# morisUtokyo/mTR

Measured on AMD Instinct MI355X. Metric: reads/sec, 2 kb Nanopore synthetic, higher is better.
Workload: dtype int32

## Files before the change

### mtr_amd/__init__.py

```python
from __future__ import annotations

import ctypes as C
import os
from typing import List, NamedTuple, Sequence

import numpy as np

HERE = os.path.dirname(os.path.abspath(__file__))
LIB_PATH = os.environ.get("MTR_LIB", os.path.join(HERE, "libmtr_hip.so"))
MAX_PERIOD = 500
MAX_READ_LENGTH = 833333
TEXT_ASCII, TEXT_CODES = 0, 1
FASTA_TILE_BYTES = 4096
FASTA_END = {0: "eof", 1: "empty", 2: "bad", 3: "toolong"}
FASTQ_END = {**FASTA_END, 4: "format", 5: "more"}

STATUS = {0: "MTR_OK", 1: "MTR_ERR_NO_DEVICE", 2: "MTR_ERR_BAD_ARG", 3: "MTR_ERR_OOM", 4: "MTR_ERR_HIP",
          5: "MTR_ERR_OVERFLOW", 6: "MTR_ERR_DP_TOO_LARGE"}
COUNTER_NAMES = ["dp_calls", "dp_cells", "dp_rows", "revise_dp_calls", "revise_dp_cells", "kmer_tables", "kmer_lookups",
                 "ranges_candidate", "ranges_executed", "records", "di_passes", "di_positions", "traceback_steps",
                 "undefined_guards", "global_tables", "reserved",
                 "cyc_total", "cyc_dp_fwd", "cyc_dp_tb", "cyc_tab_build", "cyc_seeds", "cyc_walk", "cyc_polish", "cyc_revise_vote",
                 "cyc_slot_copy", "cyc_dp_fwd_rev", "cyc_dp_tb_rev", "cyc_k1_codes", "cyc_k1_passes", "cyc_k1_extract",
                 "cyc_k1_dedup", "cyc_k1_total",
# ... 1347 lines not shown

    def last_mode(self) -> str:
        return {0: "per-read kernel", 2: "staged chain"}.get(int(self.lib.mtr_test_last_mode(self.h)), "?")

    def fetch(self) -> List[List[Record]]:
        recs = C.POINTER(CRecord)()
        cnts = C.POINTER(C.c_int32)()
        total = C.c_int64()
        self._check(self.lib.mtr_fetch_results(self.h, C.byref(recs), C.byref(cnts), C.byref(total)), "mtr_fetch_results")
        try:
            return self._unpack(recs, cnts, self.n_reads)
        finally:
            self.lib.mtr_free_results(recs, cnts)

    def process(self, reads: Sequence[np.ndarray]) -> List[List[Record]]:
        bases, offs, lens = _flatten(reads)
        recs = C.POINTER(CRecord)()
        cnts = C.POINTER(C.c_int32)()
        total = C.c_int64()
        self.n_reads = len(reads)
        self._check(self.lib.mtr_process_batch(self.h, bases.ctypes.data, offs.ctypes.data, lens.ctypes.data, len(reads),
                                               C.byref(recs), C.byref(cnts), C.byref(total)), "mtr_process_batch")
        try:
            return self._unpack(recs, cnts, len(reads))
        finally:
            self.lib.mtr_free_results(recs, cnts)

    @staticmethod
    def _unpack(recs, cnts, n) -> List[List[Record]]:
        out, p = [], 0
        for i in range(n):
            lst = []
            for _ in range(cnts[i]):
                r = recs[p]
                p += 1
                per = r.rep_period
                lst.append(Record(r.rep_start, r.rep_end, r.repeat_len, per, r.num_freq_unit, r.num_matches, r.num_mismatches,
                                  r.num_insertions, r.num_deletions, r.kmer, r.match_gain, r.mismatch_penalty, r.indel_penalty,
                                  r.unit.decode(), tuple(r.unit_score[:max(0, min(per, MAX_PERIOD))])))
            out.append(lst)
        return out

    def upload_packed(self, reads: Sequence[np.ndarray]):
        lens = np.array([len(r) for r in reads], dtype=np.int32)
        nw = lens.astype(np.int64) // 16 + 4
        woff = np.zeros(len(reads), np.int64)
        if len(reads) > 1:
            woff[1:] = np.cumsum(nw[:-1])
        packed = np.zeros(int(nw.sum()), np.uint32)
        for i, r in enumerate(reads):
            packed[woff[i]: woff[i] + nw[i]] = pack_read(np.asarray(r, np.uint8))
        self._keep = (packed, woff, lens)
        self._check(self.lib.mtr_upload_batch_packed(self.h, packed.ctypes.data, len(packed), woff.ctypes.data, lens.ctypes.data, len(reads)),
                    "mtr_upload_batch_packed")
        self.n_reads = len(reads)

    def fetch_packed(self, limit: int = -1):
        blob, cnts = C.c_void_p(), C.c_void_p()
        nbytes, total = C.c_int64(), C.c_int64()
        self._check(self.lib.mtr_fetch_results_packed(self.h, limit, C.byref(blob), C.byref(nbytes), C.byref(cnts), C.byref(total)), "mtr_fetch_results_packed")
        n = self.n_reads if limit < 0 else min(limit, self.n_reads)
        counts = np.ctypeslib.as_array(C.cast(cnts, C.POINTER(C.c_int32)), shape=(max(n, 1),))[:n].copy() if n > 0 and cnts.value else np.zeros(0, np.int32)
        data = C.string_at(blob, nbytes.value) if nbytes.value else b""
        return data, counts

    def fetch_packed_nocopy(self):
        blob, cnts = C.c_void_p(), C.c_void_p()
        nbytes, total = C.c_int64(), C.c_int64()
        self._check(self.lib.mtr_fetch_results_packed(self.h, -1, C.byref(blob), C.byref(nbytes), C.byref(cnts), C.byref(total)), "mtr_fetch_results_packed")
        return int(nbytes.value), int(total.value)

    def fetch_via_wire(self) -> List[List[Record]]:
        data, counts = self.fetch_packed()
        total = int(counts.sum())
        recs = (CRecord * max(total, 1))()
        buf = C.create_string_buffer(data, len(data)) if data else C.create_string_buffer(1)
        st = self.lib.mtr_unpack_records(buf, len(data), total, recs)
        if st != 0:
            raise MtrError(f"mtr_unpack_records: {STATUS.get(st, st)}")
        return self._unpack(recs, counts, len(counts))

    def export_packed_device(self, device_ptr: int, capacity_bytes: int):
        counts = np.zeros(self.n_reads, np.int32)
        total, nbytes = C.c_int64(), C.c_int64()
        self._check(self.lib.mtr_export_packed_device(self.h, C.c_void_p(device_ptr), capacity_bytes, counts.ctypes.data, C.byref(total), C.byref(nbytes)),
                    "mtr_export_packed_device")
        return counts, int(total.value), int(nbytes.value)

    def first_failed_read(self) -> int:
        v = C.c_int32()
        self.lib.mtr_get_first_failed_read(self.h, C.byref(v))
        return int(v.value)

    def kernel_times_ms(self):
        kt = (CKernelTime * 10)()
        self._check(self.lib.mtr_get_kernel_times(self.h, kt, 10), "mtr_get_kernel_times")
        out = {"k1_ranges": float(kt[0].ms), "k2_units": float(kt[1].ms)}
        for i, name in enumerate(("ranges", "unit_search", "alignments", "selection", "revisions", "finish_replay")):
            if kt[2 + i].launches:
                out["chain_" + name] = float(kt[2 + i].ms)
        for i, name in enumerate(("mtr_k_revise_quads", "mtr_k_dp2_quads")):
            if kt[8 + i].launches:
                out["kernel_" + name] = float(kt[8 + i].ms)
        return out

    def counters(self):
        c = (C.c_int64 * len(COUNTER_NAMES))()
        self._check(self.lib.mtr_get_counters(self.h, c, len(COUNTER_NAMES)), "mtr_get_counters")
        return {n: int(c[i]) for i, n in enumerate(COUNTER_NAMES)}

    def test_ranges(self):
        P = C.POINTER
        pc, ps, pe, pw, pd, tot = P(C.c_int32)(), P(C.c_int32)(), P(C.c_int32)(), P(C.c_int32)(), P(C.c_uint64)(), C.c_int64()
        self._check(self.lib.mtr_test_ranges(self.h, C.byref(pc), C.byref(ps), C.byref(pe), C.byref(pw), C.byref(pd), C.byref(tot)), "mtr_test_ranges")
        out, p = [], 0
        for i in range(self.n_reads):
            out.append([(ps[p + t], pe[p + t], pw[p + t], pd[p + t]) for t in range(pc[i])])
            p += pc[i]
        for ptr in (pc, ps, pe, pw, pd):
            _libc.free(C.cast(ptr, C.c_void_p))
        return out

    def test_file_tail(self):
        P = C.POINTER
        tl, to, af = P(C.c_uint16)(), P(C.c_int64)(), P(C.c_uint8)()
        self._check(self.lib.mtr_test_file_tail(self.h, C.byref(tl), C.byref(to), C.byref(af)), "mtr_test_file_tail")
        n = self.n_reads
        try:
            tail_off = np.ctypeslib.as_array(to, shape=(n + 1,)).copy()
            m = int(tail_off[n])
            tail = np.ctypeslib.as_array(tl, shape=(m,)).copy() if m else np.zeros(0, np.uint16)
            after = np.ctypeslib.as_array(af, shape=(n, 2)).copy()
        finally:
            for a in (tl, to, af):
                _libc.free(C.cast(a, C.c_void_p))
        return tail, tail_off, after

    def test_wrap_dp(self, tasks):
        n = len(tasks)
        rd = np.array([t[0] for t in tasks], np.int32)
        qs = np.array([t[1] for t in tasks], np.int32)
        qe = np.array([t[2] for t in tasks], np.int32)
        uo = np.zeros(n + 1, np.int32)
        uo[1:] = np.cumsum([len(t[3]) for t in tasks])
        units = np.ascontiguousarray(np.concatenate([np.asarray(t[3], np.uint8) for t in tasks]))
        g = np.array([t[4] for t in tasks], np.int32)
        m = np.array([t[5] for t in tasks], np.int32)
        d = np.array([t[6] for t in tasks], np.int32)
        out = np.zeros((n, 8), np.int32)
        self._check(self.lib.mtr_test_wrap_dp(self.h, n, rd.ctypes.data, qs.ctypes.data, qe.ctypes.data, units.ctypes.data, uo.ctypes.data,
                                              g.ctypes.data, m.ctypes.data, d.ctypes.data, out.ctypes.data), "mtr_test_wrap_dp")
        return out

    DP_PASSES = {"WAVE2P": 0, "Q4": 1, "QUAD2P": 2, "FOUR1P": 3, "OCT1P": 4}

    def test_wrap_dp_pass(self, dp_pass: str, groups):
        tasks = [t for g in groups for t in g]
        n = len(tasks)
        go = np.zeros(len(groups) + 1, np.int32)
        go[1:] = np.cumsum([len(g) for g in groups])
        rd = np.array([t[0] for t in tasks], np.int32)
        qs = np.array([t[1] for t in tasks], np.int32)
        qe = np.array([t[2] for t in tasks], np.int32)
        uo = np.zeros(n + 1, np.int32)
        uo[1:] = np.cumsum([len(t[3]) for t in tasks])
        units = np.ascontiguousarray(np.concatenate([np.asarray(t[3], np.uint8) for t in tasks] + [np.zeros(1, np.uint8)]))
        g = np.array([t[4] for t in tasks], np.int32)
        m = np.array([t[5] for t in tasks], np.int32)
        d = np.array([t[6] for t in tasks], np.int32)
        out = np.zeros((max(n, 1), 2, 8), np.int32)
        self._check(self.lib.mtr_test_wrap_dp_pass(self.h, self.DP_PASSES[dp_pass], len(groups), go.ctypes.data, rd.ctypes.data, qs.ctypes.data, qe.ctypes.data,
                                                   units.ctypes.data, uo.ctypes.data, g.ctypes.data, m.ctypes.data, d.ctypes.data, out.ctypes.data),
                    "mtr_test_wrap_dp_pass")
        return out[:n]

    def set_trace(self, max_events: int):
        self._check(self.lib.mtr_set_trace(self.h, max_events), "mtr_set_trace")

    def get_trace(self) -> np.ndarray:
        ev = C.POINTER(C.c_int32)()
        n = C.c_int64()
        self._check(self.lib.mtr_get_trace(self.h, C.byref(ev), C.byref(n)), "mtr_get_trace")
        arr = np.ctypeslib.as_array(ev, shape=(max(n.value, 1), 16))[: n.value].copy()
        _libc.free(C.cast(ev, C.c_void_p))
        return arr


def _c_float_text(x) -> str:
    x = float(x)
    if x != x:
        return "-nan" if np.signbit(x) else "nan"
    if x in (float("inf"), float("-inf")):
        return "inf" if x > 0 else "-inf"
    return "%f" % x


def format_report(ids, lens, report: Report, alignments: "ReportAlignments | None" = None) -> bytes:
    def host(t):
        return t.detach().cpu().numpy() if hasattr(t, "detach") else np.asarray(t)

    read, fields, ratio = host(report.read), host(report.fields).reshape(-1, 14), host(report.ratio).astype(np.float32)
    unit_off, units = host(report.unit_off), host(report.units).tobytes()
    if alignments is not None:
        col_off, text = host(alignments.col_off), np.ascontiguousarray(host(alignments.text), np.uint8)
        text = text.reshape(3, text.size // 3)
        rows = [text[0].tobytes(), text[1].tobytes(), text[2].tobytes()]
        if len(col_off) != len(read) + 1:
            raise MtrError(f"alignments of {len(col_off) - 1} repeats for a report of {len(read)}")
    out = []
    bid = [i.encode() if isinstance(i, str) else bytes(i) for i in ids]
    for k in range(len(read)):
        r = int(read[k])
        f = [int(v) for v in fields[k]]
        cols = [str(int(lens[r])), str(f[0] + 1), str(f[1] + 1), str(f[2]), str(f[3]), str(f[4]), str(f[5]), _c_float_text(ratio[k]),
                str(f[6]), str(f[7]), str(f[8])]
        out.append(bid[r] + b"\t" + "\t".join(cols).encode() + b"\t" + units[int(unit_off[k]):int(unit_off[k + 1])] + b"\n")
        if alignments is not None:
            out.append(f"\nmatch gain = {f[10]}, mismatch penalty = {f[11]}, indel penalty = {f[12]}\n\n".encode())
            c1 = int(col_off[k + 1])
            for c in range(int(col_off[k]), c1, ALIGN_WIDTH):
                e = min(c + ALIGN_WIDTH, c1)
                out.append(rows[0][c:e] + b"\n" + rows[1][c:e] + b"\n" + rows[2][c:e] + b"\n\n")
    return b"".join(out)


_COMPLEMENT = bytes.maketrans(b"ACGT", b"TGCA")


def canonical_motif(unit):
    u = unit.encode() if isinstance(unit, str) else bytes(unit)
    p = len(u)
    if p == 0:
        return unit[:0], 0, 0
    best = None
    for strand, s in enumerate((u, u.translate(_COMPLEMENT)[::-1])):
        d = s + s
        r = min(range(p), key=lambda r: (d[r:r + p], r))
        cand = (d[r:r + p], strand, r)
        if best is None or cand[0] < best[0]:
            best = cand
    canon, strand, rotation = best
    d = next(d for d in range(1, p + 1) if p % d == 0 and canon[d:] + canon[:d] == canon)
    motif = canon[:d]
    return (motif.decode() if isinstance(unit, str) else motif), strand, rotation


def format_motif_hits(ids, lens, motifs, hits: MotifHits, min_ratio: float = 0.0, min_copies: int = 1) -> bytes:
    def host(t):
        return t.detach().cpu().numpy() if hasattr(t, "detach") else np.asarray(t)

    bmot = [v.encode() if isinstance(v, str) else bytes(v) for v in motifs]
    bid = [i.encode() if isinstance(i, str) else bytes(i) for i in ids]
    n, m = len(bid), len(bmot)
    fields, score = host(hits.fields).reshape(n, m, 8), host(hits.score).reshape(n, m)
    ratio, strand = host(hits.ratio).astype(np.float32).reshape(n, m), host(hits.strand).reshape(n, m)
    if len(lens) != n:
        raise MtrError(f"{len(lens)} lengths for {n} ids")
    shown = [(b, b.translate(_COMPLEMENT)[::-1]) for b in bmot]
    out = []
    for r, k in zip(*np.nonzero((score > 0) & (ratio >= np.float32(min_ratio)) & (fields[:, :, 3] >= min_copies))):
        f = [int(v) for v in fields[r, k]]
        cols = [str(int(lens[r])), str(f[0] + 1), str(f[1] + 1), str(f[2]), str(len(bmot[k])), str(f[3]), str(f[4]), _c_float_text(ratio[r, k]),
                str(f[5]), str(f[6]), str(f[7])]
        out.append(bid[r] + b"\t" + "\t".join(cols).encode() + b"\t" + shown[k][int(strand[r, k])] + b"\n")
    return b"".join(out)


def format_motif_loci(ids, lens, motifs, loci: MotifLoci, min_ratio: float = 0.0, min_copies: int = 1) -> bytes:
    def host(t):
        return t.detach().cpu().numpy() if hasattr(t, "detach") else np.asarray(t)

    bmot = [v.encode() if isinstance(v, str) else bytes(v) for v in motifs]
    bid = [i.encode() if isinstance(i, str) else bytes(i) for i in ids]
    n, m = len(bid), len(bmot)
    off, fields = host(loci.loci_off).reshape(-1), host(loci.fields).reshape(-1, 8)
    score, ratio, strand = host(loci.score).reshape(-1), host(loci.ratio).astype(np.float32).reshape(-1), host(loci.strand).reshape(-1)
    if len(lens) != n:
        raise MtrError(f"{len(lens)} lengths for {n} ids")
    if len(off) != n * m + 1:
        raise MtrError(f"{len(off)} offsets for {n} ids and {m} motifs: {n * m + 1} needed")
    T = int(off[-1]) if len(off) else 0
    if not (len(fields) == len(score) == len(ratio) == len(strand) == T):
        raise MtrError(f"columns of {len(fields)}, {len(score)}, {len(ratio)} and {len(strand)} rows for {T} loci")
    if int(off[0]) != 0 or (np.diff(off) < 0).any():
        raise MtrError("loci_off does not ascend from 0")
    shown = [(b, b.translate(_COMPLEMENT)[::-1]) for b in bmot]
    out = []
    for p in range(n * m):
        r, k = divmod(p, m)
        for t in range(int(off[p]), int(off[p + 1])):
            f = [int(v) for v in fields[t]]
            if not (ratio[t] >= np.float32(min_ratio) and f[3] >= min_copies):
                continue
            cols = [str(int(lens[r])), str(f[0] + 1), str(f[1] + 1), str(f[2]), str(len(bmot[k])), str(f[3]), str(f[4]), _c_float_text(ratio[t]),
                    str(f[5]), str(f[6]), str(f[7])]
            out.append(bid[r] + b"\t" + "\t".join(cols).encode() + b"\t" + shown[k][int(strand[t])] + b"\n")
    return b"".join(out)


def format_flank_hits(ids, lens, patterns, hits: FlankHits, max_dist: "int | None" = None) -> bytes:
    def host(t):
        return t.detach().cpu().numpy() if hasattr(t, "detach") else np.asarray(t)

    bpat = [v.encode() if isinstance(v, str) else bytes(v) for v in patterns]
    bid = [i.encode() if isinstance(i, str) else bytes(i) for i in ids]
    n, m = len(bid), len(bpat)
    dist, start, end, strand = (host(t).reshape(n, m) for t in hits)
# ... 300 lines not shown
```

### mtr_amd/csrc/device_util.hip.inc

```
#pragma once
#include <hip/hip_runtime.h>
#include "mtr_common.h"
#include "walk_screen.h"

#define DEVINL __device__ __forceinline__

typedef __attribute__((address_space(3))) int lds_int;
typedef __attribute__((address_space(3))) unsigned char lds_u8;

DEVINL int lane_id() { return (int)(threadIdx.x & 63u); }
__device__ long long mtr_dev_wrap_dp_size = MTRC_WRAP_DP_SIZE;
DEVINL bool dp_size_ok(int U, int rows) { return (size_t)(U + 1) * (size_t)rows + (size_t)U < (size_t)mtr_dev_wrap_dp_size; }
DEVINL int uni(int v) { return __builtin_amdgcn_readfirstlane(v); }
DEVINL long long uni64(long long v)
{
    const unsigned lo = (unsigned)__builtin_amdgcn_readfirstlane((int)(unsigned)v);
    const unsigned hi = (unsigned)__builtin_amdgcn_readfirstlane((int)(unsigned)((unsigned long long)v >> 32));
    return (long long)(((unsigned long long)hi << 32) | lo);
}
DEVINL int bcast(int v, int src) { return __shfl(v, src, 64); }
DEVINL unsigned long long lanemask_lt() { return (1ull << lane_id()) - 1ull; }
DEVINL int mbcnt(unsigned long long m)
{
    return (int)__builtin_amdgcn_mbcnt_hi((unsigned)(m >> 32), __builtin_amdgcn_mbcnt_lo((unsigned)m, 0u));
// ... 65 lines not shown
{
    return __builtin_amdgcn_update_dpp(first, v, 0x111, 0xf, 0xf, false);
}
typedef unsigned short u16x2 __attribute__((ext_vector_type(2)));
DEVINL u16x2 as_pk(unsigned v) { return __builtin_bit_cast(u16x2, v); }
DEVINL unsigned as_u32(u16x2 v) { return __builtin_bit_cast(unsigned, v); }
DEVINL unsigned pk_add(unsigned a, unsigned b) { return as_u32(as_pk(a) + as_pk(b)); }
DEVINL unsigned pk_sub(unsigned a, unsigned b) { return as_u32(as_pk(a) - as_pk(b)); }
DEVINL unsigned pk_sub_sat(unsigned a, unsigned b) { return as_u32(__builtin_elementwise_sub_sat(as_pk(a), as_pk(b))); }
DEVINL unsigned max3_u32(unsigned a, unsigned b, unsigned c) { unsigned r; asm("v_max3_u32 %0, %1, %2, %3" : "=v"(r) : "v"(a), "v"(b), "v"(c)); return r; }
DEVINL unsigned pk_max(unsigned a, unsigned b) { return as_u32(__builtin_elementwise_max(as_pk(a), as_pk(b))); }
DEVINL unsigned pk_min(unsigned a, unsigned b) { return as_u32(__builtin_elementwise_min(as_pk(a), as_pk(b))); }
template <int SH>
DEVINL unsigned lshl_or(unsigned a, unsigned b)
{
    unsigned r;
    asm("v_lshl_or_b32 %0, %1, %2, %3" : "=v"(r) : "v"(a), "n"(SH), "v"(b));
    return r;
}
DEVINL unsigned pk_nonzero(unsigned a, unsigned one_pk)
{
    unsigned r;
    asm("v_pk_min_u16 %0, %1, %2" : "=v"(r) : "v"(a), "v"(one_pk));
    return r;
}

DEVINL int shift_up1(int v, int first)
{
    return __builtin_amdgcn_update_dpp(first, v, 0x138, 0xf, 0xf, false);
}

DEVINL void scan_max_first(double &v, int &idx)
{
    int lane = lane_id();
    for (int d = 1; d < 64; d <<= 1) {
        double ov = __shfl_up(v, d, 64); int oi = __shfl_up(idx, d, 64);
        if (lane >= d && !(v > ov)) { v = ov; idx = oi; }
    }
}
DEVINL void scan_min_first(double &v, int &idx)
{
    int lane = lane_id();
    for (int d = 1; d < 64; d <<= 1) {
        double ov = __shfl_up(v, d, 64); int oi = __shfl_up(idx, d, 64);
        if (lane >= d && !(v < ov)) { v = ov; idx = oi; }
    }
}

DEVINL int next_work_item(unsigned int *counter)
{
    int t = 0;
    if (lane_id() == 0) t = (int)atomicAdd(counter, 1u);
    asm volatile("" : "+v"(t));
    return __builtin_amdgcn_readfirstlane(t);
}

#define WQ_MAX 64
#define WQ_STRIDE 64
#define WQ_WORDS (WQ_MAX * WQ_STRIDE)
struct Wq { int q, nq, tried; };
DEVINL int wq_count(unsigned n) { return n >= 131072u ? 64 : n >= 32768u ? 16 : n >= 8192u ? 4 : 1; }
DEVINL void wq_init(Wq &w, unsigned n) { w.nq = wq_count(n); w.q = (int)(blockIdx.x & (unsigned)(w.nq - 1)); w.tried = 0; }
DEVINL int wq_peek_next(unsigned int *base, unsigned n, int nq, int q, unsigned B)
{
    const int lane = lane_id();
    unsigned left = 0u;
    if (lane < nq && (unsigned)lane < n) {
        const unsigned have = (n - (unsigned)lane + (unsigned)nq - 1u) / (unsigned)nq;
        const unsigned taken = __hip_atomic_load(base + lane * WQ_STRIDE, __ATOMIC_RELAXED, __HIP_MEMORY_SCOPE_AGENT);
        left = taken < have ? have - taken : 0u;
    }
    (void)B;
    const unsigned long long m = __ballot(left != 0u);
    if (m == 0ull) return -1;
    const unsigned long long behind = q < 63 ? m & (~0ull << (q + 1)) : 0ull;
    return behind != 0ull ? __builtin_ctzll(behind) : __builtin_ctzll(m);
}
DEVINL int wq_next(unsigned int *base, unsigned n, Wq &w)
{
#ifdef MTR_WQ_PEEK
    for (;;) {
        int t = 0;
        if (lane_id() == 0) t = (int)atomicAdd(base + w.q * WQ_STRIDE, 1u);
        asm volatile("" : "+v"(t));
        const unsigned long long idx = (unsigned long long)(unsigned)__builtin_amdgcn_readfirstlane(t) * (unsigned)w.nq + (unsigned)w.q;
        if (idx < (unsigned long long)n) return (int)idx;
        if (w.nq == 1) return -1;
        const int nx = wq_peek_next(base, n, w.nq, w.q, 1u);
        if (nx < 0) return -1;
        w.q = nx;
        __builtin_amdgcn_wave_barrier();
    }
#else
    int item = -1;
    while (w.tried < w.nq) {
        int t = 0;
        if (lane_id() == 0) t = (int)atomicAdd(base + w.q * WQ_STRIDE, 1u);
        asm volatile("" : "+v"(t));
        const unsigned long long idx = (unsigned long long)(unsigned)__builtin_amdgcn_readfirstlane(t) * (unsigned)w.nq + (unsigned)w.q;
        if (idx < (unsigned long long)n) { item = (int)idx; break; }
        w.q = (w.q + 1) & (w.nq - 1); w.tried++;
        __builtin_amdgcn_wave_barrier();
    }
    return item;
#endif
}

DEVINL long long wq_next_batch(unsigned int *base, unsigned n, Wq &w, unsigned B)
{
#ifndef MTR_WQ_PEEK
    long long item = -1;
    while (w.tried < w.nq) {
        int t = 0;
        if (lane_id() == 0) t = (int)atomicAdd(base + w.q * WQ_STRIDE, B);
        asm volatile("" : "+v"(t));
        const unsigned long long idx = (unsigned long long)(unsigned)__builtin_amdgcn_readfirstlane(t) * (unsigned)w.nq + (unsigned)w.q;
        if (idx < (unsigned long long)n) { item = (long long)idx; break; }
        w.q = (w.q + 1) & (w.nq - 1); w.tried++;
        __builtin_amdgcn_wave_barrier();
    }
    return item;
#endif
    for (;;) {
        int t = 0;
        if (lane_id() == 0) t = (int)atomicAdd(base + w.q * WQ_STRIDE, B);
        asm volatile("" : "+v"(t));
        const unsigned long long idx = (unsigned long long)(unsigned)__builtin_amdgcn_readfirstlane(t) * (unsigned)w.nq + (unsigned)w.q;
        if (idx < (unsigned long long)n) return (long long)idx;
        if (w.nq == 1) return -1;
        const int nx = wq_peek_next(base, n, w.nq, w.q, B);
        if (nx < 0) return -1;
        w.q = nx;
        __builtin_amdgcn_wave_barrier();
    }
}

DEVINL void loop_join() { __builtin_amdgcn_wave_barrier(); }

DEVINL void count_add(unsigned long long *counters, int which, long long v)
{
    if (lane_id() == 0) atomicAdd(&counters[which], (unsigned long long)v);
}
DEVINL void wc_add(unsigned long long *wc, int which, long long v)
{
    if (lane_id() == 0) wc[which] += (unsigned long long)v;
}
#ifdef MTR_PROFILE
DEVINL unsigned long long clk() { return __builtin_amdgcn_s_memtime(); }
DEVINL void wc_time(unsigned long long *wc, int which, unsigned long long t0) { wc_add(wc, which, (long long)(clk() - t0)); }
#else
DEVINL unsigned long long clk() { return 0ull; }
DEVINL void wc_time(unsigned long long *, int, unsigned long long) {}
#endif
#ifdef MTR_PROFILE_WALK_FMT
#define wc_time_aux(wc, which, t0) do { } while (0)
#else
#define wc_time_aux(wc, which, t0) wc_time(wc, which, t0)
#endif
DEVINL void wc_flush(unsigned long long *wc, unsigned long long *global)
{
    const int lane = lane_id();
    __builtin_amdgcn_wave_barrier();
    if (lane < CNT_N) { unsigned long long v = wc[lane]; if (v) atomicAdd(&global[lane], v); wc[lane] = 0ull; }
    __builtin_amdgcn_wave_barrier();
}
DEVINL void set_status(int32_t *status, int code)
{
    if (lane_id() == 0) atomicCAS(status, 0, code);
}
DEVINL void wave_sync_mem()
{
    __builtin_amdgcn_fence(__ATOMIC_RELEASE, "workgroup");
    __builtin_amdgcn_wave_barrier();
    __builtin_amdgcn_fence(__ATOMIC_ACQUIRE, "workgroup");
}
```

### mtr_amd/csrc/dp_quad.hip.inc

```
#pragma once
#include "device_util.hip.inc"

struct DpQuad {
    const uint32_t *pk[4];
    long long wlim[4];
    int base[4], rows[4], U[4];
    const uint8_t *unit[4];
    int n;
    int G[4], MM[4], D[4];
};
#define DPQ_SCALE 4
#define DPQ_FITS_SC(SC, rows, U, G, D) ((long)(SC) * ((long)(rows) * (long)(G) + (long)(D) * ((long)(U) + 2)) < 65000L)
#define DPQ_FITS(rows, U, G, D) DPQ_FITS_SC(DPQ_SCALE, rows, U, G, D)
#define DPQ_COLS(U) (((U) + 15) >> 4)
#define DPQ_COLS64(U) (((U) + 63) >> 6)
#define DPQ_ROW_BYTES_G(GL, C) ((GL) * (C))
#define DPQ_DP_BYTES_G(GL, C, maxrows) ((size_t)(maxrows) * DPQ_ROW_BYTES_G(GL, C) + 16)
#define DPQ_ROW_BYTES(C) DPQ_ROW_BYTES_G(16, C)
#define DPQ_DP_BYTES(C, maxrows) DPQ_DP_BYTES_G(16, C, maxrows)
#define DPQ_BLOCK_BYTES(C, maxrows) (4 * DPQ_DP_BYTES(C, maxrows))
#define DPQP_DP_BYTES_G(GL, C, maxrows) ((size_t)(((maxrows) + 1) >> 1) * DPQ_ROW_BYTES_G(GL, C) + 16)
#define DPQP_DP_BYTES(C, maxrows) DPQP_DP_BYTES_G(16, C, maxrows)
#define DPQP_BLOCK_BYTES(C, maxrows) (4 * DPQP_DP_BYTES(C, maxrows))

template <int C, int GL = 16, int SC = DPQ_SCALE>
DEVINL void dp_forward2p_g16(const DpQuad &q, int G0, int MM0, int D0, int G1, int MM1, int D1, uint8_t *cells, int maxrows, int (&best)[4][2][3])
{
    static_assert(C >= 1 && C <= 8 && (GL == 16 || GL == 64) && (SC == 1 || SC == 4), "columns per lane, lanes per DP, score scale");
    constexpr int NG = 64 / GL;
    const int lane = lane_id();
    const int g = lane / GL, l = lane % GL;
    unsigned Gpk = SC * ((unsigned)G0 | ((unsigned)G1 << 16)), MMpk = SC * ((unsigned)MM0 | ((unsigned)MM1 << 16)), Dpk = SC * ((unsigned)D0 | ((unsigned)D1 << 16));
    unsigned ONE = 0x00010001u, TWO = 0x00020002u, FOUR = 0x00040004u, SEL_HI = 0x07060100u, C8 = 0x00080008u;
    asm volatile("" : "+v"(ONE), "+v"(TWO), "+v"(FOUR), "+v"(SEL_HI), "+v"(C8));
    unsigned SEL_K0 = 0x0c040100u, SEL_K1 = 0x0c040302u, SEL_S = 0x05040100u, SEL_LO = 0x05040100u, SEL_P1 = 0x07060302u, K4N = ~0x00040004u;
    asm volatile("" : "+s"(MMpk), "+s"(Dpk), "+s"(SEL_K0), "+s"(SEL_K1), "+s"(SEL_S), "+s"(SEL_LO), "+s"(SEL_P1), "+s"(K4N));
    int Ul = q.U[0], basel = q.base[0], rowsl = q.rows[0]; const uint8_t *up_ = q.unit[0]; const uint32_t *pkl = q.pk[0]; long long wl = q.wlim[0];
    if (g == 1) { Ul = q.U[1]; basel = q.base[1]; rowsl = q.rows[1]; up_ = q.unit[1]; pkl = q.pk[1]; wl = q.wlim[1]; }
    if (g == 2) { Ul = q.U[2]; basel = q.base[2]; rowsl = q.rows[2]; up_ = q.unit[2]; pkl = q.pk[2]; wl = q.wlim[2]; }
    if (g == 3) { Ul = q.U[3]; basel = q.base[3]; rowsl = q.rows[3]; up_ = q.unit[3]; pkl = q.pk[3]; wl = q.wlim[3]; }
    if (g >= q.n) { Ul = 0; rowsl = 0; }
    unsigned ubw[2] = { 0x04040404u, 0x04040404u };
    unsigned Kc[C], KGc[C];
#pragma unroll
    for (int c = 0; c < C; c++) {
        const int j = l * C + c + 1;
        if (j <= Ul) ubw[c >> 2] = (ubw[c >> 2] & ~(0xffu << (8 * (c & 3)))) | ((unsigned)(up_[j - 1] & 3) << (8 * (c & 3)));
        Kc[c] = SC * ((unsigned)(D0 * (c + 1)) | ((unsigned)(D1 * (c + 1)) << 16));
        KGc[c] = Kc[c] + Gpk;
    }
    const unsigned Dlane = SC * ((unsigned)(D0 * l * C) | ((unsigned)(D1 * l * C) << 16));
    {
        int landed = lane_val((int)(ubw[0] ^ ubw[1]), 0);
        asm volatile("" :: "s"(landed));
    }
    const int lU = Ul > 0 ? (Ul - 1) / C : 0, rU = Ul > 0 ? (Ul - 1) % C : 0;
    const int hu_addr = (g * GL + lU) << 2;
    const int lUs = GL == 64 ? uni(lU) : 0;
    bool is_r[C];
#pragma unroll
    for (int c = 0; c < C; c++) is_r[c] = rU == c;
    const bool lane0 = l == 0;
    const int grp_addr = (g * GL) << 2;
    constexpr bool BKP = SC == 4;
    static_assert(65000 / DPQ_SCALE <= 0x7FFF, "DPQ_FITS must keep the rows of an SC = 4 pass within the 15 bits of the pair keys");
    constexpr int NBK = BKP ? (C + 1) / 2 : C;
    unsigned P[C], bk0[NBK], bk1[NBK];
#pragma unroll
    for (int c = 0; c < C; c++) P[c] = 0u;
#pragma unroll
    for (int c = 0; c < NBK; c++) { bk0[c] = 0u; bk1[c] = 0u; }
    unsigned wrapv = 0u;
    int next_done = maxrows + 1;
#pragma unroll
    for (int h = 0; h < NG; h++) { const int r = h < q.n ? q.rows[h] : 0; if (r < next_done) next_done = r; }
    if (rowsl <= 0) { ubw[0] = 0x04040404u; ubw[1] = 0x04040404u; }
    uint8_t *crow = cells + (size_t)g * DPQ_DP_BYTES_G(GL, C, maxrows) + (size_t)l * C;
    int i = 1;
    constexpr int CHUNK = 16 * GL - 16;
    for (int t0 = 0; t0 < maxrows; t0 += CHUNK) {
        const int pos0 = basel + 1 + t0;
        long long w0 = (long long)(pos0 >> 4) + l;
        long long w1 = w0 + 1;
        if (w0 > wl - 1) w0 = wl - 1;
        if (w1 > wl - 1) w1 = wl - 1;
        if (w0 < 0) w0 = 0;
        if (w1 < 0) w1 = 0;
        const uint32_t wa = pkl[w0], wb = pkl[w1];
        const unsigned sh = 2u * (unsigned)(pos0 & 15);
        const uint32_t A = (uint32_t)(((((unsigned long long)wa) << 32) | (unsigned long long)wb) >> (32u - sh));
        {
            int landed = lane_val((int)A, 0);
            asm volatile("" :: "s"(landed));
        }
        const int i_chunk_end = t0 + CHUNK < maxrows ? t0 + CHUNK : maxrows;
        for (int wd = 0; i <= i_chunk_end; wd++) {
            const uint32_t wcur = (uint32_t)__builtin_amdgcn_ds_bpermute(grp_addr + (wd << 2), (int)A);
            const int i_w_end = i + 15 < i_chunk_end ? i + 15 : i_chunk_end;
            int bsh = 30;
#pragma unroll 1
            for (; i <= i_w_end; i++, bsh -= 2) {
                if (i > next_done) {
                    if (i > rowsl) { ubw[0] = 0x04040404u; ubw[1] = 0x04040404u; }
                    next_done = maxrows + 1;
#pragma unroll
                    for (int h = 0; h < NG; h++) { const int r = h < q.n ? q.rows[h] : 0; if (r >= i && r < next_done) next_done = r; }
                }
                const unsigned xi = __builtin_amdgcn_ubfe(wcur, (unsigned)bsh, 2u);
                const unsigned inv_i = 0xFFFFu - (unsigned)i;
                unsigned s[C], t1s[C];
                bool mt[C], nh[C];
                unsigned sprev = 0u;
                bool nhp = true;
                const unsigned diag0 = GL == 16 ? (unsigned)row_shift_up1((int)P[C - 1], (int)wrapv) : (unsigned)shift_up1((int)P[C - 1], (int)wrapv);
#pragma unroll
                for (int c = 0; c < C; c++) {
                    const unsigned diag = c == 0 ? diag0 : P[c - 1];
                    const unsigned upv = P[c];
                    const bool m = ((ubw[c >> 2] >> (8 * (c & 3))) & 0xffu) == xi;
                    const unsigned t1 = pk_sub_sat(diag, MMpk), t2 = pk_sub_sat(upv, Dpk);
                    const unsigned gnm = pk_max(t1, t2) + Kc[c];
                    const unsigned gm = diag + KGc[c];
                    const unsigned ch = pk_max(gnm, sprev);
                    const unsigned sc = m ? gm : ch;
                    s[c] = sc; t1s[c] = t1; mt[c] = m;
                    nhp = nhp && !m; nh[c] = nhp;
                    sprev = sc;
                }
                const unsigned long long hm = __ballot(!nhp);
                const unsigned seg = (unsigned)mbcnt(hm >> 1);
                const unsigned sout = sprev + Dlane;
                unsigned k0 = __builtin_amdgcn_perm(seg, sout, SEL_K0);
                unsigned k1 = __builtin_amdgcn_perm(seg, sout, SEL_K1);
                if (GL == 16) scan_max_u32_x2_row16(k0, k1); else scan_max_u32_x2(k0, k1);
                const unsigned S = __builtin_amdgcn_perm(k1, k0, SEL_S);
                const unsigned e = (GL == 16 ? (unsigned)row_shift_up1((int)S, 0) : (unsigned)shift_up1((int)S, 0)) - Dlane;
                unsigned f[8];
#pragma unroll
                for (int c = C; c < 8; c++) f[c] = 0u;
                unsigned hgp = e;
#pragma unroll
                for (int c = 0; c < C; c++) {
                    const unsigned mx = pk_max(s[c], e);
                    const unsigned hg = nh[c] ? mx : s[c];
                    const unsigned H = hg - Kc[c];
                    const unsigned nz = pk_nonzero(H, ONE);
                    const unsigned nx = pk_nonzero(H - t1s[c], SC == 4 ? TWO : ONE);
                    const unsigned nd = pk_nonzero(hg - hgp, SC == 4 ? FOUR : ONE);
                    unsigned fl;
                    if (SC == 4) asm("v_or3_b32 %0, %1, %2, %3" : "=v"(fl) : "v"(nz), "v"(nx), "v"(nd));
                    else fl = lshl_or<1>(nx, lshl_or<2>(nd, nz));
                    fl = mt[c] ? C8 : fl;
                    f[c] = fl;
                    if (!BKP) {
                        const unsigned q0 = (H << 16) | inv_i, q1 = __builtin_amdgcn_perm(H, inv_i, SEL_HI);
                        bk0[c] = q0 > bk0[c] ? q0 : bk0[c];
                        bk1[c] = q1 > bk1[c] ? q1 : bk1[c];
                    }
                    P[c] = H;
                    hgp = hg;
                }
                if (BKP) {
                    const unsigned r0 = (0x7FFFu - (unsigned)i) << 1, r1 = r0 | 1u;
#pragma unroll
                    for (int c = 0; c + 1 < C; c += 2) {
                        const unsigned a0 = (P[c] << 16) | r1, b0 = (P[c + 1] << 16) | r0;
                        const unsigned a1 = __builtin_amdgcn_perm(P[c], r1, SEL_HI), b1 = __builtin_amdgcn_perm(P[c + 1], r0, SEL_HI);
                        bk0[c >> 1] = max3_u32(bk0[c >> 1], a0, b0);
                        bk1[c >> 1] = max3_u32(bk1[c >> 1], a1, b1);
                    }
                    if (C & 1) {
                        const unsigned a0 = (P[C - 1] << 16) | r1, a1 = __builtin_amdgcn_perm(P[C - 1], r1, SEL_HI);
                        bk0[C >> 1] = a0 > bk0[C >> 1] ? a0 : bk0[C >> 1];
                        bk1[C >> 1] = a1 > bk1[C >> 1] ? a1 : bk1[C >> 1];
                    }
                }
                unsigned hsel = P[0];
#pragma unroll
                for (int c = 1; c < C; c++) hsel = is_r[c] ? P[c] : hsel;
                wrapv = GL == 64 ? (unsigned)__builtin_amdgcn_readlane((int)hsel, lUs) : (unsigned)__builtin_amdgcn_ds_bpermute(hu_addr, (int)hsel);
                {
                    unsigned nd0 = pk_nonzero(pk_sub(pk_add(P[0], Dpk), wrapv), SC == 4 ? FOUR : ONE);
                    if (SC != 4) nd0 <<= 2;
                    unsigned f0;
                    asm("v_and_or_b32 %0, %1, %2, %3" : "=v"(f0) : "v"(f[0]), "s"(K4N), "v"(nd0));
                    f[0] = (lane0 && !mt[0]) ? f0 : f[0];
                }
                const unsigned F01 = lshl_or<8>(f[1], f[0]), F23 = lshl_or<8>(f[3], f[2]);
                unsigned lo = lshl_or<4>(__builtin_amdgcn_perm(F23, F01, SEL_P1), __builtin_amdgcn_perm(F23, F01, SEL_LO));
                if (C > 4) {
                    const unsigned F45 = C > 5 ? lshl_or<8>(f[5], f[4]) : f[4], F67 = C > 7 ? lshl_or<8>(f[7], f[6]) : f[6];
                    unsigned hi = lshl_or<4>(__builtin_amdgcn_perm(F67, F45, SEL_P1), __builtin_amdgcn_perm(F67, F45, SEL_LO));
                    if (C < 8) {
                        const unsigned nlo = (unsigned)__builtin_amdgcn_update_dpp(0, (int)lo, 0x130, 0xf, 0xf, false);
                        hi = lshl_or<8 * (C > 4 && C < 8 ? C - 4 : 0)>(nlo, hi);
                    }
                    *(uint2 *)crow = make_uint2(lo, hi);
                } else if (C == 1) {
                    *crow = (uint8_t)lo;
                } else {
                    if (C < 4) {
                        const unsigned nlo = (unsigned)__builtin_amdgcn_update_dpp(0, (int)lo, 0x130, 0xf, 0xf, false);
                        lo = lshl_or<8 * (C < 4 ? C : 0)>(nlo, lo);
                    }
                    *(uint32_t *)crow = lo;
                }
                crow += DPQ_ROW_BYTES_G(GL, C);
                loop_join();
            }
            loop_join();
        }
        loop_join();
    }
#pragma unroll
    for (int d = 0; d < 2; d++) {
        int v = 0, vi = 0, vj = 0;
#pragma unroll
        for (int t = 0; t < NBK; t++) {
            const unsigned bk = d == 0 ? bk0[t] : bk1[t];
            const int c = BKP ? 2 * t + 1 - (int)(bk & 1u) : t;
            const int j = l * C + c + 1;
            const int bvc = (int)(bk >> 16), bic = BKP ? (int)(0x7FFFu - ((bk & 0xFFFFu) >> 1)) : (int)(0xFFFFu - (bk & 0xFFFFu));
            if (j <= Ul && (bvc > v || (bvc == v && bvc > 0 && bic < vi))) { v = bvc; vi = bic; vj = j; }
        }
        for (int dd = GL / 2; dd > 0; dd >>= 1) {
            const int ov = __shfl_xor(v, dd, 64), oi = __shfl_xor(vi, dd, 64), oj = __shfl_xor(vj, dd, 64);
            const bool take = (ov > v) || (ov == v && ov > 0 && (oi < vi || (oi == vi && oj < vj)));
            if (take) { v = ov; vi = oi; vj = oj; }
        }
#pragma unroll
        for (int h = 0; h < NG; h++) { best[h][d][0] = lane_val(v, GL * h) / SC; best[h][d][1] = lane_val(vi, GL * h); best[h][d][2] = lane_val(vj, GL * h); }
    }
}


DEVINL unsigned u16_max(unsigned a, unsigned b) { unsigned r; asm("v_max_u16_e32 %0, %1, %2" : "=v"(r) : "v"(a), "v"(b)); return r; }
DEVINL unsigned u16_min(unsigned a, unsigned b) { unsigned r; asm("v_min_u16_e32 %0, %1, %2" : "=v"(r) : "v"(a), "v"(b)); return r; }
DEVINL unsigned u16_sub_sat(unsigned a, unsigned b) { unsigned r; asm("v_sub_u16_e64 %0, %1, %2 clamp" : "=v"(r) : "v"(a), "v"(b)); return r; }
DEVINL unsigned u16_sub(unsigned a, unsigned b) { unsigned r; asm("v_sub_u16_e32 %0, %1, %2" : "=v"(r) : "v"(a), "v"(b)); return r; }
DEVINL unsigned scan_max_u32_row16(unsigned a)
{
    unsigned s;
#define MTR_SCAN_STEP(ctrl) s = (unsigned)__builtin_amdgcn_update_dpp(0, (int)a, ctrl, 0xf, 0xf, false); a = s > a ? s : a;
    MTR_SCAN_STEP(0x111) MTR_SCAN_STEP(0x112) MTR_SCAN_STEP(0x114) MTR_SCAN_STEP(0x118)
#undef MTR_SCAN_STEP
    return a;
}
template <int C, int GL = 16, int SC = DPQ_SCALE, bool PAIR = false>
DEVINL void dp_forward1p_g16(const DpQuad &q, uint8_t *cells, int maxrows, int (&best)[4][3])
{
    static_assert(C >= 1 && C <= 8 && (GL == 16 || GL == 64) && (SC == 1 || SC == 4), "columns per lane, lanes per DP, score scale");
    constexpr int NG = 64 / GL;
    const int lane = lane_id();
    const int g = lane / GL, l = lane % GL;
    unsigned ONE = 1u, TWO = 2u, FOUR = 4u, EIGHT = 8u;
    asm volatile("" : "+v"(ONE), "+v"(TWO), "+v"(FOUR), "+v"(EIGHT));
    int Ul = q.U[0], basel = q.base[0], rowsl = q.rows[0]; const uint8_t *up_ = q.unit[0]; const uint32_t *pkl = q.pk[0]; long long wl = q.wlim[0];
    int Gl = q.G[0], MMl = q.MM[0], Dl = q.D[0];
    if (g == 1) { Ul = q.U[1]; basel = q.base[1]; rowsl = q.rows[1]; up_ = q.unit[1]; pkl = q.pk[1]; wl = q.wlim[1]; Gl = q.G[1]; MMl = q.MM[1]; Dl = q.D[1]; }
    if (g == 2) { Ul = q.U[2]; basel = q.base[2]; rowsl = q.rows[2]; up_ = q.unit[2]; pkl = q.pk[2]; wl = q.wlim[2]; Gl = q.G[2]; MMl = q.MM[2]; Dl = q.D[2]; }
    if (g == 3) { Ul = q.U[3]; basel = q.base[3]; rowsl = q.rows[3]; up_ = q.unit[3]; pkl = q.pk[3]; wl = q.wlim[3]; Gl = q.G[3]; MMl = q.MM[3]; Dl = q.D[3]; }
    if (g >= q.n) { Ul = 0; rowsl = 0; }
    const unsigned Gs = SC * (unsigned)Gl, MMs = SC * (unsigned)MMl, Ds = SC * (unsigned)Dl;
    unsigned ubw[2] = { 0x04040404u, 0x04040404u };
    unsigned Dj[C], GDj[C];
#pragma unroll
    for (int c = 0; c < C; c++) {
        const int j = l * C + c + 1;
        if (j <= Ul) ubw[c >> 2] = (ubw[c >> 2] & ~(0xffu << (8 * (c & 3)))) | ((unsigned)(up_[j - 1] & 3) << (8 * (c & 3)));
        Dj[c] = Ds * (unsigned)j;
        GDj[c] = Dj[c] + Gs;
    }
    {
        int landed = lane_val((int)(ubw[0] ^ ubw[1]), 0);
        asm volatile("" :: "s"(landed));
    }
    const int lU = Ul > 0 ? (Ul - 1) / C : 0, rU = Ul > 0 ? (Ul - 1) % C : 0;
    const int hu_addr = (g * GL + lU) << 2;
    const int lUs = GL == 64 ? uni(lU) : 0;
    bool is_r[C];
#pragma unroll
    for (int c = 0; c < C; c++) is_r[c] = rU == c;
    const bool lane0 = l == 0;
    const int grp_addr = (g * GL) << 2;
    constexpr bool BKP = SC == 4;
    constexpr int NBK = BKP ? (C + 1) / 2 : C;
    unsigned P[C], bk[NBK];
#pragma unroll
    for (int c = 0; c < C; c++) P[c] = 0u;
#pragma unroll
    for (int c = 0; c < NBK; c++) bk[c] = 0u;
    unsigned wrapv = 0u;
    int next_done = maxrows + 1;
#pragma unroll
    for (int h = 0; h < NG; h++) { const int r = h < q.n ? q.rows[h] : 0; if (r < next_done) next_done = r; }
    if (rowsl <= 0) { ubw[0] = 0x04040404u; ubw[1] = 0x04040404u; }
    uint8_t *crow = cells + (size_t)g * (PAIR ? DPQP_DP_BYTES_G(GL, C, maxrows) : DPQ_DP_BYTES_G(GL, C, maxrows)) + (size_t)l * C;
    unsigned loP = 0u, hiP = 0u;
    auto store_cells = [&](unsigned lo, unsigned hi) {
        if (C > 4) {
            if (C < 8) {
                const unsigned nlo = (unsigned)__builtin_amdgcn_update_dpp(0, (int)lo, 0x130, 0xf, 0xf, false);
                hi |= nlo << (8 * (C > 4 && C < 8 ? C - 4 : 0));
            }
            *(uint2 *)crow = make_uint2(lo, hi);
        } else if (C == 1) {
            *crow = (uint8_t)lo;
        } else {
            if (C < 4) {
                const unsigned nlo = (unsigned)__builtin_amdgcn_update_dpp(0, (int)lo, 0x130, 0xf, 0xf, false);
                lo |= nlo << (8 * (C < 4 ? C : 0));
            }
            *(uint32_t *)crow = lo;
        }
        crow += DPQ_ROW_BYTES_G(GL, C);
    };
    int i = 1;
    constexpr int CHUNK = 16 * GL - 16;
    for (int t0 = 0; t0 < maxrows; t0 += CHUNK) {
        const int pos0 = basel + 1 + t0;
        long long w0 = (long long)(pos0 >> 4) + l;
        long long w1 = w0 + 1;
        if (w0 > wl - 1) w0 = wl - 1;
        if (w1 > wl - 1) w1 = wl - 1;
        if (w0 < 0) w0 = 0;
        if (w1 < 0) w1 = 0;
        const uint32_t wa = pkl[w0], wb = pkl[w1];
        const unsigned sh = 2u * (unsigned)(pos0 & 15);
        const uint32_t A = (uint32_t)(((((unsigned long long)wa) << 32) | (unsigned long long)wb) >> (32u - sh));
        {
            int landed = lane_val((int)A, 0);
            asm volatile("" :: "s"(landed));
        }
        const int i_chunk_end = t0 + CHUNK < maxrows ? t0 + CHUNK : maxrows;
        for (int wd = 0; i <= i_chunk_end; wd++) {
            const uint32_t wcur = (uint32_t)__builtin_amdgcn_ds_bpermute(grp_addr + (wd << 2), (int)A);
            const int i_w_end = i + 15 < i_chunk_end ? i + 15 : i_chunk_end;
            int bsh = 30;
#pragma unroll 1
            for (; i <= i_w_end; i++, bsh -= 2) {
                if (i > next_done) {
                    if (i > rowsl) { ubw[0] = 0x04040404u; ubw[1] = 0x04040404u; }
                    next_done = maxrows + 1;
#pragma unroll
                    for (int h = 0; h < NG; h++) { const int r = h < q.n ? q.rows[h] : 0; if (r >= i && r < next_done) next_done = r; }
                }
                const unsigned xi = __builtin_amdgcn_ubfe(wcur, (unsigned)bsh, 2u);
                const unsigned inv_i = 0xFFFFu - (unsigned)i;
                unsigned s[C], t1s[C];
                bool mt[C], nh[C];
                unsigned sprev = 0u;
                bool nhp = true;
                const unsigned diag0 = GL == 16 ? (unsigned)row_shift_up1((int)P[C - 1], (int)wrapv) : (unsigned)shift_up1((int)P[C - 1], (int)wrapv);
#pragma unroll
                for (int c = 0; c < C; c++) {
                    const unsigned diag = c == 0 ? diag0 : P[c - 1];
                    const unsigned upv = P[c];
                    const bool m = ((ubw[c >> 2] >> (8 * (c & 3))) & 0xffu) == xi;
                    const unsigned t1 = u16_sub_sat(diag, MMs), t2 = u16_sub_sat(upv, Ds);
                    const unsigned gnm = u16_max(t1, t2) + Dj[c];
                    const unsigned gm = diag + GDj[c];
                    const unsigned ch = u16_max(gnm, sprev);
                    const unsigned sc = m ? gm : ch;
                    s[c] = sc; t1s[c] = t1; mt[c] = m;
                    nhp = nhp && !m; nh[c] = nhp;
                    sprev = sc;
                }
                const unsigned long long hm = __ballot(!nhp);
                const unsigned seg = (unsigned)mbcnt(hm >> 1);
                const unsigned S = (GL == 16 ? scan_max_u32_row16((seg << 16) | sprev) : scan_max_u32((seg << 16) | sprev)) & 0xFFFFu;
                const unsigned e = GL == 16 ? (unsigned)row_shift_up1((int)S, 0) : (unsigned)shift_up1((int)S, 0);
                unsigned f[8];
#pragma unroll
                for (int c = C; c < 8; c++) f[c] = 0u;
                unsigned hgp = e;
#pragma unroll
                for (int c = 0; c < C; c++) {
                    const unsigned mx = u16_max(s[c], e);
                    const unsigned hg = nh[c] ? mx : s[c];
                    const unsigned H = hg - Dj[c];
                    const unsigned nz = u16_min(H, ONE);
                    const unsigned nx = u16_min(H - t1s[c], SC == 4 ? TWO : ONE);
                    const unsigned nd = u16_min(hg - hgp, SC == 4 ? FOUR : ONE);
                    unsigned fl = SC == 4 ? (nz | nx | nd) : (nz | (nx << 1) | (nd << 2));
// ... 295 lines not shown
```

### mtr_amd/csrc/dp_test.hip.inc

```
#pragma once
#include "dp_wrap.hip.inc"

struct DpPassArgs {
    DpTestArgs t;
    int32_t pass, n_groups;
    const int32_t *group_off;
    long long packed_words;
};

DEVINL void dpt_clear(DpRes &o) { o.stop_i = 0; o.end_i = 0; o.mat = o.mis = o.ins = o.del = o.scanned = 0; o.end_j = 0; }
DEVINL void dpt_store(const DpPassArgs &a, int task, int p, int qs, int U, const DpRes &o)
{
    if (lane_id() == 0) {
        int32_t *r = a.t.out8 + ((size_t)task * 2 + (size_t)p) * 8;
        r[0] = qs + o.stop_i + 1; r[1] = qs + o.end_i; r[2] = o.end_i - o.stop_i; r[3] = U > 0 ? o.scanned / U : 0;
        r[4] = o.mat; r[5] = o.mis; r[6] = o.ins; r[7] = o.del;
    }
}
template <int FMT>
DEVINL void dpt_traceback(const DpPassArgs &a, const uint32_t *pk, int qs, int U, const uint8_t *cells, int psel, int rstride, const int (&best)[3],
                          DpRes &o, unsigned long long *wc)
{
    dpt_clear(o);
    const int bv = uni(best[0]), bi = uni(best[1]), bj = uni(best[2]);
    if (bv > 0) {
        dp_traceback<0, FMT>(pk, qs, U, cells, psel, rstride, bi, bj, nullptr, nullptr, nullptr, o, wc);
        if (o.stop_i < 0) { dpt_clear(o); set_status(a.t.status, DEV_ERR_DP_TOO_LARGE); }
    }
}

__global__ __launch_bounds__(64, MTR_DP2_WAVES_PER_SIMD) void mtr_k_dp_test_waves(DpPassArgs a)
{
    __shared__ unsigned long long s_cnt[CNT_N];
    if (lane_id() < CNT_N) s_cnt[lane_id()] = 0ull;
    uint8_t *sc = a.t.scratch + (size_t)blockIdx.x * a.t.scratch_per_wave;
    for (;;) {
        const int grp = next_work_item(a.t.work_counter);
        if (grp >= a.n_groups) break;
        const int t0 = uni(a.group_off[grp]), n = uni(a.group_off[grp + 1]) - t0;
        const int rd = uni(a.t.read_idx[t0]);
        const uint32_t *pk = a.t.b.packed + uni64(a.t.b.woff[rd]);
        const int qs = uni(a.t.qs[t0]), rows = uni(a.t.qe[t0]) - qs + 1;
        if (a.pass == MTR_TEST_PASS_WAVE2P) {
            const int uo = uni(a.t.unit_off[t0]), U = uni(a.t.unit_off[t0 + 1]) - uo;
            const uint8_t *unit = a.t.units + uo;
            DpRes o[2];
            bool ok;
            if (dp_wrap2_fits(rows, U, a.t.dp16_max_rows)) ok = dp_wrap2(pk, qs, rows, unit, U, 1, 1, 3, 1, 3, 1, sc, a.t.cells_cap, o, s_cnt, a.t.dp16_max_rows);
            else {
                ok = dp_wrap(pk, qs, rows, unit, U, 1, 1, 3, sc, a.t.cells_cap, 0, nullptr, nullptr, nullptr, o[0], s_cnt, a.t.dp16_max_rows);
                ok = dp_wrap(pk, qs, rows, unit, U, 1, 3, 1, sc, a.t.cells_cap, 0, nullptr, nullptr, nullptr, o[1], s_cnt, a.t.dp16_max_rows) && ok;
            }
            if (!ok) set_status(a.t.status, DEV_ERR_DP_TOO_LARGE);
            dpt_store(a, t0, 0, qs, U, o[0]); dpt_store(a, t0, 1, qs, U, o[1]);
        } else {
            Dp4 q; q.n = n;
            size_t off = 0;
#pragma unroll
            for (int g = 0; g < 4; g++) {
                const bool on = g < n;
                const int tg = t0 + (on ? g : 0);
                const int uo = uni(a.t.unit_off[tg]);
                q.U[g] = on ? uni(a.t.unit_off[tg + 1]) - uo : 1; q.unit[g] = a.t.units + uo;
                q.off[g] = on ? off : 0;
                if (on) off += (size_t)rows * (size_t)q.U[g];
            }
            int best[4][2][3];
            dp_forward2p_q4(pk, qs, rows, q, 1, 1, 3, 1, 3, 1, sc, best);
            wave_sync_mem();
#pragma unroll
            for (int g = 0; g < 4; g++) {
                if (g < n) {
                    for (int p = 0; p < 2; p++) {
                        DpRes o;
                        dpt_traceback<1>(a, pk, qs, q.U[g], sc + q.off[g], p, q.U[g], best[g][p], o, s_cnt);
                        dpt_store(a, t0 + g, p, qs, q.U[g], o);
                        loop_join();
                    }
                }
            }
        }
        wave_sync_mem();
        loop_join();
    }
    wc_flush(s_cnt, a.t.counters);
}

template <int C>
__global__ __launch_bounds__(64, 4) void mtr_k_dp_test_quads(DpPassArgs a)
{
    __shared__ unsigned long long s_cnt[CNT_N];
    if (lane_id() < CNT_N) s_cnt[lane_id()] = 0ull;
    uint8_t *cells = a.t.scratch + (size_t)blockIdx.x * a.t.scratch_per_wave;
    for (;;) {
        const int grp = next_work_item(a.t.work_counter);
        if (grp >= a.n_groups) break;
        const int t0 = uni(a.group_off[grp]), n = uni(a.group_off[grp + 1]) - t0;
        DpQuad q; q.n = n;
        int maxrows = 0;
#pragma unroll
        for (int g = 0; g < 4; g++) {
            const int tg = t0 + (g < n ? g : 0);
            const int rd = uni(a.t.read_idx[tg]), uo = uni(a.t.unit_off[tg]);
            q.pk[g] = a.t.b.packed + uni64(a.t.b.woff[rd]);
            q.wlim[g] = a.packed_words - uni64(a.t.b.woff[rd]);
            q.base[g] = uni(a.t.qs[tg]); q.rows[g] = g < n ? uni(a.t.qe[tg]) - q.base[g] + 1 : 0;
            q.U[g] = uni(a.t.unit_off[tg + 1]) - uo; q.unit[g] = a.t.units + uo;
            q.G[g] = 1; q.MM[g] = 1; q.D[g] = 1;
            maxrows = q.rows[g] > maxrows ? q.rows[g] : maxrows;
        }
        int best[4][2][3];
        dp_forward2p_g16<C>(q, 1, 1, 3, 1, 3, 1, cells, maxrows, best);
        wave_sync_mem();
#pragma unroll
        for (int g = 0; g < 4; g++) {
            if (g < n) {
                for (int p = 0; p < 2; p++) {
                    DpRes o;
                    dpt_traceback<1>(a, q.pk[g], q.base[g], q.U[g], cells + g * DPQ_DP_BYTES(C, maxrows), p, DPQ_ROW_BYTES(C), best[g][p], o, s_cnt);
                    dpt_store(a, t0 + g, p, q.base[g], q.U[g], o);
                    loop_join();
                }
            }
        }
        wave_sync_mem();
        loop_join();
    }
    wc_flush(s_cnt, a.t.counters);
}

__global__ __launch_bounds__(64, MTR_WAVES_PER_SIMD) void mtr_k_dp_test_rev(DpPassArgs a)
{
    __shared__ unsigned long long s_cnt[CNT_N];
    if (lane_id() < CNT_N) s_cnt[lane_id()] = 0ull;
    uint8_t *cells = a.t.scratch + (size_t)blockIdx.x * a.t.scratch_per_wave;
    for (;;) {
        const int grp = next_work_item(a.t.work_counter);
        if (grp >= a.n_groups) break;
        const int t0 = uni(a.group_off[grp]), n = uni(a.group_off[grp + 1]) - t0;
        DpOct q; q.n = n;
        int maxrows = 0, maxU = 0;
#pragma unroll 1
        for (int g = 0; g < RQ_SLOTS; g++) { q.pk[g] = a.t.b.packed; q.wlim[g] = 1; q.base[g] = 0; q.rows[g] = 0; q.U[g] = 0; q.unit[g] = cells; q.G[g] = 1; q.MM[g] = 1; q.D[g] = 1; }
#pragma unroll 1
        for (int k = 0; k < n; k++) {
            const int tg = t0 + k;
            const int rd = uni(a.t.read_idx[tg]), uo = uni(a.t.unit_off[tg]);
            q.pk[k] = a.t.b.packed + uni64(a.t.b.woff[rd]); q.wlim[k] = a.packed_words - uni64(a.t.b.woff[rd]);
            q.base[k] = uni(a.t.qs[tg]); q.rows[k] = uni(a.t.qe[tg]) - q.base[k] + 1;
            q.U[k] = uni(a.t.unit_off[tg + 1]) - uo; q.unit[k] = a.t.units + uo;
            q.G[k] = uni(a.t.gain[tg]); q.MM[k] = uni(a.t.mism[tg]); q.D[k] = uni(a.t.indel[tg]);
            maxrows = q.rows[k] > maxrows ? q.rows[k] : maxrows; maxU = q.U[k] > maxU ? q.U[k] : maxU;
        }
        const int Cq = DPQ_COLS(maxU);
        int best[RQ_SLOTS][3];
        for (int g = 0; g < RQ_SLOTS; g++) { best[g][0] = 0; best[g][1] = 0; best[g][2] = 0; }
        if (a.pass == MTR_TEST_PASS_FOUR1P) st_fwd1p_four(Cq, q, cells, maxrows, best); else st_fwd1p_any(Cq, q, cells, maxrows, best);
        wave_sync_mem();
#pragma unroll 1
        for (int k = 0; k < n; k++) {
            int bk[3] = { best[0][0], best[0][1], best[0][2] };
#pragma unroll
            for (int h = 1; h < RQ_SLOTS; h++) if (k == h) { bk[0] = best[h][0]; bk[1] = best[h][1]; bk[2] = best[h][2]; }
            const int tg = t0 + k;
            const int rd = uni(a.t.read_idx[tg]), qs = uni(a.t.qs[tg]), U = uni(a.t.unit_off[tg + 1]) - uni(a.t.unit_off[tg]);
            DpRes o;
            dpt_traceback<3>(a, a.t.b.packed + uni64(a.t.b.woff[rd]), qs, U, cells + (size_t)k * DPQP_DP_BYTES(Cq, maxrows), 0, DPQ_ROW_BYTES(Cq), bk, o, s_cnt);
            dpt_store(a, tg, 0, qs, U, o);
            loop_join();
        }
        wave_sync_mem();
        loop_join();
    }
    wc_flush(s_cnt, a.t.counters);
}
```

### mtr_amd/csrc/k3_staged.hip.inc

```
#pragma once
#include "k2_units.hip.inc"
#include "dp_quad.hip.inc"

#define ST_QCLASSES 8
#define ST_QROWBINS 2048
#define ST_QSUB 8
#define ST_NBINS (ST_QCLASSES * ST_QROWBINS * ST_QSUB)
#define ST_QUMAX 128

struct StItemHdr {
    int32_t n_slots; uint32_t run_mask, found_mask; int32_t min_k, max_k;
    int32_t rd, t, qs, qe, w, item, stride;
    long long pad0, pad1;
};
struct StEnt { int32_t period, k, dir, dpi; };
struct StK { int32_t state, slot; int32_t rr[14]; long long rev_off; };
struct StRev { long long block; int32_t k, slot; int32_t rr[14]; long long leader; int32_t ri, pad[3]; };
#define ST_REV_BYTES ((long long)sizeof(StRev) + K2_SLOT_UNIT + 4ll * K2_SLOT_SCORE)
struct StDpItem { int32_t rd, qs, rows, U; long long unit_off, codes_off; int32_t best[6]; int32_t pad[2]; };
static_assert(sizeof(StItemHdr) == 64 && sizeof(StEnt) == 16 && sizeof(StDpItem) == 64 && sizeof(StK) == 72 && sizeof(StRev) == 96, "staged layouts");

struct StagedArgs {
    int32_t n_reads;
    int64_t *item_off; int32_t *n_items;
    int4 *item_tab; int32_t item_cap;
    uint8_t *arena; long long arena_cap;
    long long *kc_items; int32_t kc_cap;
    long long *rb_items;
    StDpItem *dp; int32_t dp_cap;
    unsigned *bin_count; int32_t *dp_bin, *dp_rank;
    int32_t *bin_start; int32_t *sorted; int32_t sorted_cap; int32_t *quad_cls;
    int32_t quad_min;
    DevRecord *cand; int32_t cand_cap; unsigned *n_cand; int32_t *cand_flag;
    unsigned *work;
    int4 *cont; int32_t cont_cap;
    int32_t k_first;
    long long *rev_items; int32_t rev_cap; unsigned *n_rev;
    int32_t *wv_items; int32_t *dp_res;
    int32_t nsub;
    int32_t two_pass, pass, defer_w;
    int32_t pass_shuffle;
    int32_t test_flags;
    int8_t *item_pass; int32_t *pass_list[2]; unsigned *n_pass[2];
    int32_t *re2;
    int32_t walk_screen; int32_t *walk_list; int32_t walk_cap; unsigned *n_walk;
};

#define ST_NCLS 8
#define ST_CLS_STRIDE 64
DEVINL int st_cost_class(int rows)
{
    if (rows < 128) return 0;
    const int c = (31 - __builtin_clz((unsigned)rows)) - 6;
    return c > ST_NCLS - 1 ? ST_NCLS - 1 : c;
}
#define ST_Q_DP 16
#define ST_Q_WK 24
#define ST_Q_REV 32
#define ST_Q_QUAD 40
#define ST_Q_POLISH 56
#define ST_N_QUEUES 64
#define ST_WQ(s, j) ((s).work + (size_t)(j) * WQ_WORDS)
DEVINL bool st_staged_overflowed(const K2Args &a) { return uni(*(volatile int32_t *)a.status) == DEV_ERR_STAGED_OVERFLOW; }

#define ST_SL_DP 1
#define ST_SL_ARENA 2
#define ST_SL_KC 3
#define ST_SL_REV 4
#define ST_SL_RB 58
#define ST_DPI_DUP 0x40000000
DEVINL int st_sl_cont(int cls) { return cls < 2 ? 6 + cls : cls == 2 ? 9 : 11 + (cls - 3); }
#define ST_SL_WV 48
DEVINL unsigned *st_sub(const StagedArgs &s, int slot, int q) { return ST_WQ(s, slot) + (size_t)q * WQ_STRIDE; }
DEVINL int st_my_sub(const StagedArgs &s) { return (int)(blockIdx.x & (unsigned)(s.nsub - 1)); }
DEVINL long long st_reserve(const StagedArgs &s, int slot, long long cap, unsigned n)
{
    const int q = st_my_sub(s);
    const long long per = cap / s.nsub;
    unsigned got = 0;
    if (lane_id() == 0) got = atomicAdd(st_sub(s, slot, q), n);
    got = (unsigned)uni((int)got);
    if ((long long)got + (long long)n > per) return -1;
    return (long long)q * per + (long long)got;
}
DEVINL long long st_reserve_bytes(const StagedArgs &s, long long bytes)
{
    const int q = st_my_sub(s);
    const long long per = (s.arena_cap / s.nsub) & ~15ll;
    unsigned long long got = 0;
    if (lane_id() == 0) got = atomicAdd((unsigned long long *)st_sub(s, ST_SL_ARENA, q), (unsigned long long)bytes);
    got = (unsigned long long)uni64((long long)got);
    if ((long long)got + bytes > per) return -1;
    return (long long)q * per + (long long)got;
}
struct WqS { int q, tried, cnt; };
DEVINL long long wqs_init(WqS &w, const StagedArgs &s, int cslot, long long cap)
{
    const int lane = lane_id();
    const long long per = cap / s.nsub;
    unsigned c = lane < s.nsub ? *st_sub(s, cslot, lane) : 0u;
    if ((long long)c > per) c = (unsigned)per;
    w.cnt = (int)c; w.q = st_my_sub(s); w.tried = 0;
    return wave_sum_i64((long long)c);
}
DEVINL long long wqs_next(const StagedArgs &s, int qslot, long long cap, WqS &w)
{
    const long long per = cap / s.nsub;
#ifndef MTR_WQ_PEEK
    while (w.tried < s.nsub) {
        const int n_q = lane_val(w.cnt, w.q);
        if (n_q > 0) {
            int t = 0;
            if (lane_id() == 0) t = (int)atomicAdd(ST_WQ(s, qslot) + (size_t)w.q * WQ_STRIDE, 1u);
            asm volatile("" : "+v"(t));
            t = __builtin_amdgcn_readfirstlane(t);
            if (t < n_q) return (long long)w.q * per + (long long)t;
        }
        w.q = (w.q + 1) & (s.nsub - 1); w.tried++;
        __builtin_amdgcn_wave_barrier();
    }
    return -1;
#endif
    for (;;) {
        const int n_q = lane_val(w.cnt, w.q);
        if (n_q > 0) {
            int t = 0;
            if (lane_id() == 0) t = (int)atomicAdd(ST_WQ(s, qslot) + (size_t)w.q * WQ_STRIDE, 1u);
            asm volatile("" : "+v"(t));
            t = __builtin_amdgcn_readfirstlane(t);
            if (t < n_q) return (long long)w.q * per + (long long)t;
        }
        if (s.nsub == 1) return -1;
        unsigned left = 0u;
        if (lane_id() < s.nsub) {
            const unsigned taken = __hip_atomic_load(ST_WQ(s, qslot) + (size_t)lane_id() * WQ_STRIDE, __ATOMIC_RELAXED, __HIP_MEMORY_SCOPE_AGENT);
            left = taken < (unsigned)w.cnt ? (unsigned)w.cnt - taken : 0u;
        }
        const unsigned long long m = __ballot(left != 0u);
        if (m == 0ull) return -1;
        const unsigned long long behind = w.q < 63 ? m & (~0ull << (w.q + 1)) : 0ull;
        w.q = behind != 0ull ? __builtin_ctzll(behind) : __builtin_ctzll(m);
        __builtin_amdgcn_wave_barrier();
    }
}
DEVINL long long st_pad16(long long x) { return (x + 15) & ~15ll; }

__global__ __launch_bounds__(1024) void mtr_k_items(const int32_t *r_count, StagedArgs s)
{
    __shared__ long long part[1024];
    const int tid = (int)threadIdx.x, n = s.n_reads;
    const int per = (n + 1023) / 1024;
    const int lo = tid * per, hi = lo + per < n ? lo + per : n;
    long long sum = 0;
    for (int i = lo; i < hi; i++) sum += r_count[i];
    part[tid] = sum;
    __syncthreads();
    for (int d = 1; d < 1024; d <<= 1) {
        const long long v = tid >= d ? part[tid - d] : 0;
        __syncthreads();
        part[tid] += v;
        __syncthreads();
// ... 272 lines not shown
                    for (int k = k_last + 1; k <= max_k; k++)
                        if ((alive >> (k - min_k)) & 1u) s.cont[q++] = make_int4((int)(unsigned)(base & 0xffffffffll), (int)(base >> 32), k, bound);
                }
                wave_sync_mem();
                st_park_entries(c, s, base, st, min_k, stride, n_slots, maxU);
            }
        }
        loop_join();
        }
        loop_join();
    }
    wc_flush(s_cnt, a.counters);
}

__global__ __launch_bounds__(64, MTR_WAVES_PER_SIMD) void mtr_k_walks_k(K2Args a, StagedArgs s)
{
    __shared__ __attribute__((aligned(16))) int s_arena[MTR_ARENA_INTS];
    __shared__ unsigned long long s_cnt[CNT_N];
    int *s_keys = s_arena, *s_seeds = s_arena + K2_TAB_CAP, *s_stage = s_seeds + MTRC_MAX_SEEDS + 4;
    const int lane = lane_id();
    if (lane < CNT_N) s_cnt[lane] = 0ull;
    if (st_staged_overflowed(a)) return;
    K2Ctx c;
    c.a = &a; c.wc = s_cnt; c.staged_walks = true;
#ifdef MTR_PROFILE_WALK_FMT
    c.prof_kernel = 1;
#endif
    c.sc = a.scratch + (size_t)blockIdx.x * a.scratch_per_wave;
    c.y = k2_layout(a.Lmax, a.cells_cap);
    c.lds_keys = (lds_int *)s_keys; c.seeds = (lds_int *)s_seeds; c.stage = (lds_int *)s_stage;
    c.ties = (int *)(c.sc + c.y.ties); c.fresh = c.ties + MTRC_MAX_TIEBREAKS;
    for (int cls = ST_NCLS - 1; cls >= 0; cls--) {
    WqS wq;
    if (wqs_init(wq, s, st_sl_cont(cls), s.cont_cap) == 0) continue;
    for (;;) {
        const long long wi = wqs_next(s, ST_Q_WK + cls, s.cont_cap, wq);
        if (wi < 0) break;
        int4 rec = make_int4(0, 0, 0, 0);
        if (lane == 0) rec = s.cont[(size_t)cls * (size_t)s.cont_cap + wi];
        const long long base = (long long)(((unsigned long long)(unsigned)uni(rec.y) << 32) | (unsigned)uni(rec.x));
        const int k = uni(rec.z), bound = uni(rec.w);
        StItemHdr *h = (StItemHdr *)(s.arena + base);
        c.rd = uni(h->rd);
        const int qs = uni(h->qs), qe = uni(h->qe), w = uni(h->w), min_k = uni(h->min_k), n_slots = uni(h->n_slots), stride = uni(h->stride);
        c.L = uni(a.b.lens[c.rd]);
        c.pk = a.b.packed + uni64(a.b.woff[c.rd]);
        c.memo_n = 0; c.memo_qs = c.memo_qe = -1; c.memo_U = 0;
        RangeP1 st;
#ifdef MTR_PROFILE_WALK_WIDTH
        const unsigned long long t_w = clk();
#endif
        k2_range_walks(c, qs, qe, w, st, k, k, bound);
#ifdef MTR_PROFILE_WALK_WIDTH
        { const int wd_ = qe - qs + 1; wc_time(c.wc, wd_ < 32 ? CNT_SPARE43 : wd_ < 64 ? CNT_SPARE44 : wd_ < 128 ? CNT_SPARE45 : wd_ < 256 ? CNT_SPARE46 : CNT_SPARE55, t_w); }
#endif
        if (lane == 0) { if (st.run_mask) atomicOr(&h->run_mask, st.run_mask); if (st.found_mask) atomicOr(&h->found_mask, st.found_mask); }
        if (st.n_ent > 0) st_park_entries(c, s, base, st, min_k, stride, n_slots, st_max_unit(qs, qe));
        loop_join();
    }
    loop_join();
    }
    wc_flush(s_cnt, a.counters);
}

DEVINL unsigned st_rotl(unsigned x, int r) { return (x << r) | (x >> (32 - r)); }
__global__ __launch_bounds__(64) void mtr_k_gather(K2Args a, StagedArgs s)
{
    const int lane = lane_id();
    if (st_staged_overflowed(a)) return;
    WqS wq; (void)wqs_init(wq, s, ST_SL_KC, s.kc_cap);
    for (;;) {
        const long long wi = wqs_next(s, 8, s.kc_cap, wq);
        if (wi < 0) break;
        const long long base = uni64(s.kc_items[wi]);
        StItemHdr *h = (StItemHdr *)(s.arena + base);
        StEnt *en = (StEnt *)(h + 1);
        int hv = 0;
        if (lane < 12) hv = ((const int32_t *)h)[lane];
        const int n_slots = lane_val(hv, 0), min_k = lane_val(hv, 3), rd = lane_val(hv, 5), qs = lane_val(hv, 7), qe = lane_val(hv, 8), stride = lane_val(hv, 11);
        const unsigned found_mask = (unsigned)lane_val(hv, 2);
        const int rows = qe - qs + 1;
        const int ns = n_slots < 32 ? n_slots : 32;
        int Ue = 0, ke = min_k;
        if (lane < ns) { Ue = en[lane].period; ke = en[lane].k; }
        uint8_t *slot0 = s.arena + base + (long long)sizeof(StItemHdr) + (long long)sizeof(StEnt) * n_slots;
        const bool cand_l = lane < ns && Ue >= MTRC_MIN_PERIOD && ((found_mask >> (ke - min_k)) & 1u);
        const unsigned candm = (unsigned)__ballot(cand_l);
        if (candm == 0u) { loop_join(); continue; }
        unsigned h1 = 0u, h2 = 0u;
        if (cand_l) {
            const uint32_t *uw = (const uint32_t *)(slot0 + (long long)lane * stride);
            const int nw = (Ue + 3) >> 2;
            const uint32_t last_mask = (Ue & 3) ? ((1u << (8 * (Ue & 3))) - 1u) : 0xffffffffu;
            int q = 0;
            for (; q + 4 <= nw; q += 4) {
                uint32_t w0 = uw[q], w1 = uw[q + 1], w2 = uw[q + 2], w3 = uw[q + 3];
                if (q + 4 == nw) w3 &= last_mask;
                h1 = st_rotl((h1 ^ w0) * 0x9E3779B1u, 13); h2 = (h2 + w0) * 0x85EBCA77u; h2 ^= h2 >> 15;
                h1 = st_rotl((h1 ^ w1) * 0x9E3779B1u, 13); h2 = (h2 + w1) * 0x85EBCA77u; h2 ^= h2 >> 15;
                h1 = st_rotl((h1 ^ w2) * 0x9E3779B1u, 13); h2 = (h2 + w2) * 0x85EBCA77u; h2 ^= h2 >> 15;
                h1 = st_rotl((h1 ^ w3) * 0x9E3779B1u, 13); h2 = (h2 + w3) * 0x85EBCA77u; h2 ^= h2 >> 15;
            }
            for (; q < nw; q++) {
                uint32_t w0 = uw[q];
                if (q + 1 == nw) w0 &= last_mask;
                h1 = st_rotl((h1 ^ w0) * 0x9E3779B1u, 13); h2 = (h2 + w0) * 0x85EBCA77u; h2 ^= h2 >> 15;
            }
        }
        unsigned want = 0u;
        int dupof_l = -1;
        for (unsigned cm = candm; cm != 0u; cm &= cm - 1u) {
            const int e = __builtin_ctz(cm);
            const int U = lane_val(Ue, e);
            const unsigned e1 = (unsigned)lane_val((int)h1, e), e2 = (unsigned)lane_val((int)h2, e);
            const uint8_t *ub = slot0 + (long long)e * stride;
            bool dup = false;
            for (unsigned sm = (unsigned)__ballot(lane < ns && Ue == U && h1 == e1 && h2 == e2) & want; sm != 0u && !dup; sm &= sm - 1u) {
                const int j = __builtin_ctz(sm);
                const uint8_t *u2 = slot0 + (long long)j * stride;
                bool diff = false;
                for (int q = lane; q < U; q += 64) diff = diff || (u2[q] != ub[q]);
                dup = __ballot(diff) == 0ull;
                if (dup && lane == e) dupof_l = j;
                loop_join();
            }
            if (!dup) want |= 1u << e;
            loop_join();
        }
        const int n_want = __builtin_popcount(want);
        const bool fits16 = rows <= DP2P_MAX_ROWS && rows <= a.dp16_max_rows;
        const bool grouping = fits16 && s.dp_cap < (1 << 28);
        const bool isq = s.quad_min > 0 && fits16 && Ue <= ST_QUMAX && DPQ_FITS(rows, Ue, 1, 3) && dp_size_ok(Ue, rows);
        const unsigned quadm = (unsigned)__ballot(isq) & want, smallm = (unsigned)__ballot(!isq && grouping && Ue <= 16) & want;
        const unsigned restm = want & ~smallm & ~quadm;
        const int n_small = __builtin_popcount(smallm), n_quad = __builtin_popcount(quadm), n_entries = (n_small + 3) / 4 + (n_want - n_small - n_quad);
        const int cls = st_cost_class(rows);
        const long long dres = st_reserve(s, ST_SL_DP, s.dp_cap, (unsigned)n_want);
        const long long wres = n_entries > 0 ? st_reserve(s, ST_SL_WV + cls, s.dp_cap, (unsigned)n_entries) : 0;
        if (dres < 0 || wres < 0) { set_status(a.status, DEV_ERR_STAGED_OVERFLOW); loop_join(); continue; }
        const unsigned di0 = (unsigned)dres, wv0 = (unsigned)wres;
        int dpi_l = -1;
        if (lane < 32 && ((want >> lane) & 1u)) {
            const unsigned below = (1u << lane) - 1u;
            const bool is_small = (smallm >> lane) & 1u, is_quad = (quadm >> lane) & 1u;
            const int nth = is_small ? __builtin_popcount(smallm & below) : is_quad ? n_small + __builtin_popcount(quadm & below) : n_small + n_quad + __builtin_popcount(restm & below);
            const unsigned di = di0 + (unsigned)nth;
            dpi_l = (int)di;
            StDpItem *d = s.dp + di;
            d->rd = rd; d->qs = qs; d->rows = rows; d->U = Ue; d->unit_off = (long long)(slot0 + (long long)lane * stride - s.arena); d->codes_off = -1;
            for (int q = 0; q < 6; q++) d->best[q] = 0;
            d->pad[0] = ke; d->pad[1] = cls;
            if (is_quad) {
                int rb = ST_QROWBINS - 1 - (rows >> 3); if (rb < 0) rb = 0;
                const int bin = ((8 - DPQ_COLS(Ue)) * ST_QROWBINS + rb) * ST_QSUB + (int)(blockIdx.x & (ST_QSUB - 1));
                s.dp_bin[di] = bin; s.dp_rank[di] = (int32_t)atomicAdd(s.bin_count + bin, 1u);
            } else {
                s.dp_bin[di] = -1;
                if (is_small) {
                    if ((nth & 3) == 0) {
                        const int members = n_small - nth < 4 ? n_small - nth : 4;
                        s.wv_items[(size_t)cls * (size_t)s.dp_cap + wv0 + (unsigned)(nth >> 2)] = (int32_t)(di | ((unsigned)(members - 1) << 28));
                    }
                } else s.wv_items[(size_t)cls * (size_t)s.dp_cap + wv0 + (unsigned)((n_small + 3) / 4 + (nth - n_small - n_quad))] = (int32_t)di;
            }
            en[lane].dpi = (int32_t)di;
        }
        {
            const int od = __shfl(dpi_l, dupof_l >= 0 ? dupof_l : 0, 64);
            if (dupof_l >= 0 && od >= 0 && s.dp_cap < ST_DPI_DUP) en[lane].dpi = (int32_t)(od | ST_DPI_DUP);
        }
        wave_sync_mem();
        loop_join();
    }
}

__global__ __launch_bounds__(1024) void mtr_k_qbins(StagedArgs s, int force)
{
    __shared__ int tot[1024];
    __shared__ int cls_start[ST_QCLASSES + 1], cls_n[ST_QCLASSES];
    const int t = (int)threadIdx.x;
    constexpr int PER = ST_NBINS / 1024, TPC = ST_QROWBINS * ST_QSUB / PER;
    static_assert(PER % 4 == 0, "a thread's bins are read four at a time");
    int sum = 0;
    for (int r = 0; r < PER; r += 4) { const uint4 v = *(const uint4 *)(s.bin_count + t * PER + r); sum += (int)(v.x + v.y + v.z + v.w); }
    tot[t] = sum;
    __syncthreads();
    for (int d = 1; d < 1024; d <<= 1) {
        const int v = t >= d ? tot[t - d] : 0;
        __syncthreads();
        tot[t] += v;
        __syncthreads();
    }
    if (t == 0) {
        int off = 0;
        for (int c = 0; c < ST_QCLASSES; c++) {
            const int n = tot[(c + 1) * TPC - 1] - (c > 0 ? tot[c * TPC - 1] : 0);
            cls_start[c] = off; cls_n[c] = n;
            off += (n + 3) & ~3;
        }
        cls_start[ST_QCLASSES] = off;
        const bool use = s.quad_min > 0 && (force || tot[1023] >= s.quad_min) && off <= s.sorted_cap;
        for (int c = 0; c <= ST_QCLASSES; c++) s.quad_cls[c] = use ? cls_start[c] : 0;
        s.quad_cls[ST_QCLASSES + 1] = use ? 1 : 0;
        if (use) for (int c = 0; c < ST_QCLASSES; c++) for (int q = cls_start[c] + cls_n[c]; q < cls_start[c + 1]; q++) s.sorted[q] = -1;
    }
    __syncthreads();
    const int c = t / TPC;
    int off = cls_start[c] + (tot[t] - sum) - (c > 0 ? tot[c * TPC - 1] : 0);
    for (int r = 0; r < PER; r += 4) {
        const uint4 v = *(const uint4 *)(s.bin_count + t * PER + r);
        int4 o; o.x = off; o.y = off + (int)v.x; o.z = o.y + (int)v.y; o.w = o.z + (int)v.z;
        *(int4 *)(s.bin_start + t * PER + r) = o;
        off = o.w + (int)v.w;
        *(uint4 *)(s.bin_count + t * PER + r) = make_uint4(0u, 0u, 0u, 0u);
    }
}
__global__ void mtr_k_qscatter(StagedArgs s, int32_t *status)
{
    if (*(volatile int32_t *)status == DEV_ERR_STAGED_OVERFLOW) return;
    const unsigned per = (unsigned)(s.dp_cap / s.nsub);
    const bool use = s.quad_cls[ST_QCLASSES + 1] != 0;
    for (unsigned i = blockIdx.x * blockDim.x + threadIdx.x; i < per * (unsigned)s.nsub; i += gridDim.x * blockDim.x) {
        if (i % per >= *st_sub(s, ST_SL_DP, (int)(i / per))) continue;
        if (s.dp_bin[i] < 0) continue;
        if (use) {
            const int slot = s.bin_start[s.dp_bin[i]] + s.dp_rank[i];
            if (slot >= 0 && slot < s.sorted_cap) s.sorted[slot] = (int32_t)i;
        } else {
            const int cls = s.dp[i].pad[1];
            const unsigned wper = (unsigned)(s.dp_cap / s.nsub), wq_ = blockIdx.x & (unsigned)(s.nsub - 1);
            const unsigned w = atomicAdd(st_sub(s, ST_SL_WV + cls, (int)wq_), 1u);
            if (w < wper) s.wv_items[(size_t)cls * (size_t)s.dp_cap + (size_t)wq_ * wper + w] = (int32_t)i;
            else atomicCAS(status, 0, DEV_ERR_STAGED_OVERFLOW);
        }
    }
}

__global__ void mtr_k_rscatter(StagedArgs s, int32_t *status)
{
    if (*(volatile int32_t *)status == DEV_ERR_STAGED_OVERFLOW) return;
    const unsigned per = (unsigned)(s.rev_cap / s.nsub);
    for (unsigned i = blockIdx.x * blockDim.x + threadIdx.x; i < per * (unsigned)s.nsub; i += gridDim.x * blockDim.x) {
        if (i % per >= *st_sub(s, ST_SL_REV, (int)(i / per))) continue;
        if (s.dp_bin[i] < 0) continue;
        const int slot = s.bin_start[s.dp_bin[i]] + s.dp_rank[i];
        if (slot >= 0 && slot < s.sorted_cap) s.sorted[slot] = (int32_t)i;
    }
}

DEVINL void st_dp2_waves_body(K2Ctx &c, const K2Args &a, const StagedArgs &s)
{
    const int lane = lane_id();
    for (int cls = ST_NCLS - 1; cls >= 0; cls--) {
    WqS wq;
    if (wqs_init(wq, s, ST_SL_WV + cls, s.dp_cap) == 0) continue;
    for (;;) {
        const long long wi = wqs_next(s, ST_Q_DP + cls, s.dp_cap, wq);
        if (wi < 0) break;
        const unsigned ent = (unsigned)uni(s.wv_items[(size_t)cls * (size_t)s.dp_cap + wi]);
        const int di0 = (int)(ent & 0x0FFFFFFFu), members = (int)(ent >> 28) + 1;
        const StDpItem *d0 = s.dp + di0;
        c.rd = uni(d0->rd);
        c.L = uni(a.b.lens[c.rd]);
        c.pk = a.b.packed + uni64(a.b.woff[c.rd]);
        const int qs = uni(d0->qs), rows = uni(d0->rows);
        if (members > 1 && dp_batch_fits(c, rows)) {
            Dp4 q; q.n = members;
            int kk[4];
#pragma unroll
            for (int g = 0; g < 4; g++) {
                const StDpItem *dg = s.dp + di0 + (g < members ? g : 0);
                q.U[g] = uni(dg->U); kk[g] = uni(dg->pad[0]); q.unit[g] = s.arena + uni64(dg->unit_off); q.off[g] = 0;
            }
            dp_two_params_q4(c, qs, qs + rows - 1, q, kk, [&](int g, const RR &r, bool) {
                int *o = s.dp_res + (size_t)(di0 + g) * 16;
                if (lane == 0) {
                    o[0] = r.rep_start; o[1] = r.rep_end; o[2] = r.repeat_len; o[3] = r.period; o[4] = r.copies; o[5] = r.mat; o[6] = r.mis;
                    o[7] = r.ins; o[8] = r.del; o[9] = r.kmer; o[10] = r.G; o[11] = r.MM; o[12] = r.D;
                }
            });
        } else {
        for (int g = 0; g < members; g++) {
        const int di = di0 + g;
        const StDpItem *d = s.dp + di;
        const int U = uni(d->U);
        RR r; rr_clear(r); r.period = U; r.kmer = uni(d->pad[0]);
        dp_two_params_unit(c, qs, qs + rows - 1, r, s.arena + uni64(d->unit_off));
        int *o = s.dp_res + (size_t)di * 16;
        if (lane == 0) {
            o[0] = r.rep_start; o[1] = r.rep_end; o[2] = r.repeat_len; o[3] = r.period; o[4] = r.copies; o[5] = r.mat; o[6] = r.mis;
            o[7] = r.ins; o[8] = r.del; o[9] = r.kmer; o[10] = r.G; o[11] = r.MM; o[12] = r.D;
        }
        loop_join();
        }
        }
        loop_join();
    }
    loop_join();
    }
}
#ifndef MTR_DP2_WAVES_PER_SIMD
#define MTR_DP2_WAVES_PER_SIMD 8
#endif
__global__ __launch_bounds__(64, MTR_DP2_WAVES_PER_SIMD) void mtr_k_dp2_waves(K2Args a, StagedArgs s)
{
    __shared__ unsigned long long s_cnt[CNT_N];
    const int lane = lane_id();
    if (lane < CNT_N) s_cnt[lane] = 0ull;
    if (st_staged_overflowed(a)) return;
    K2Ctx c;
    c.a = &a; c.wc = s_cnt;
    c.sc = a.scratch + (size_t)blockIdx.x * a.scratch_per_wave;
    c.y = k2_layout(a.Lmax, a.cells_cap);
    c.lds_keys = nullptr; c.seeds = nullptr; c.stage = nullptr; c.ties = nullptr; c.fresh = nullptr;
    st_dp2_waves_body(c, a, s);
    wc_flush(s_cnt, a.counters);
}

template <int C>
DEVINL void st_quad_run(K2Ctx &c, const K2Args &a, const StagedArgs &s, const int (&items)[4], DpQuad &q, const int (&kk)[4], int maxrows)
{
    const int lane = lane_id();
    uint8_t *cells = c.sc + c.y.codes;
    int best[4][2][3];
    const unsigned long long t_f = clk();
    dp_forward2p_g16<C>(q, 1, 1, 3, 1, 3, 1, cells, maxrows, best);
    wave_sync_mem();
    wc_time(c.wc, CYC_DP_FWD, t_f);
    if (lane == 0) {
        unsigned long long served = 0ull;
        for (int g = 0; g < q.n; g++) served += (unsigned long long)q.rows[g] * (unsigned long long)q.U[g];
        c.wc[CNT_QPASS_BYTES_DP2] += 4ull * (unsigned long long)maxrows * (unsigned long long)DPQ_ROW_BYTES(C);
        c.wc[CNT_QPASS_CELLS_DP2] += served;
    }
    const unsigned long long t_b = clk();
#pragma unroll
    for (int g = 0; g < 4; g++) {
        if (g < q.n) {
            const int U = q.U[g], qs = q.base[g], rows = q.rows[g];
            c.rd = uni(s.dp[items[g]].rd);
            RR r; rr_clear(r); r.period = U; r.kmer = kk[g];
            RR bestr; rr_clear(bestr);
            float best_ratio = -1.0f;
            long long tb = 0;
            bool ok = true;
            for (int p = 0; p < 2; p++) {
                DpRes o; o.stop_i = 0; o.end_i = 0; o.mat = o.mis = o.ins = o.del = o.scanned = 0; o.end_j = 0;
                const int bv = uni(best[g][p][0]), bi = uni(best[g][p][1]), bj = uni(best[g][p][2]);
                if (bv > 0) {
                    dp_traceback<0, 1>(q.pk[g], qs, U, cells + g * DPQ_DP_BYTES(C, maxrows), p, DPQ_ROW_BYTES(C), bi, bj, nullptr, nullptr, nullptr, o, c.wc);
                    if (o.stop_i < 0) { o.stop_i = 0; o.end_i = 0; o.mat = o.mis = o.ins = o.del = o.scanned = 0; ok = false; }
                }
                tb += (long long)(o.mat + o.mis + o.ins + o.del);
                RR t = r;
                apply_dp(t, qs, o, U, 1, p == 0 ? 1 : 3, p == 0 ? 3 : 1);
                trace_ev(c, 3, qs, qs + rows - 1, U, trace_on(c, 3) ? unit_hash(q.unit[g], U) : 0, 1, p == 0 ? 1 : 3, p == 0 ? 3 : 1, t.rep_start, t.rep_end, t.repeat_len, t.copies, t.mat, t.mis, t.ins);
                const float qq = rr_ratio(t);
                if (best_ratio < qq) { bestr = t; best_ratio = qq; }
                loop_join();
            }
            if (!ok) { dp_too_large(c); rr_clear(bestr); }
            int *o = s.dp_res + (size_t)items[g] * 16;
            if (lane == 0) {
                o[0] = bestr.rep_start; o[1] = bestr.rep_end; o[2] = bestr.repeat_len; o[3] = bestr.period; o[4] = bestr.copies; o[5] = bestr.mat; o[6] = bestr.mis;
                o[7] = bestr.ins; o[8] = bestr.del; o[9] = bestr.kmer; o[10] = bestr.G; o[11] = bestr.MM; o[12] = bestr.D;
                c.wc[CNT_DP_CALLS] += 2ull; c.wc[CNT_DP_CELLS] += 2ull * (unsigned long long)rows * (unsigned long long)U;
                c.wc[CNT_DP_ROWS] += 2ull * (unsigned long long)rows; c.wc[CNT_TB_STEPS] += (unsigned long long)tb;
            }
        }
    }
    wc_time(c.wc, CYC_DP_TB, t_b);
    wave_sync_mem();
}
DEVINL unsigned st_scatter_stride(unsigned n)
{
    if (n < 4u) return 1u;
    unsigned s = (unsigned)(0.6180339887 * (double)n) | 1u;
    for (;;) {
        unsigned x = n, y = s;
        while (y != 0u) { const unsigned t = x % y; x = y; y = t; }
        if (x == 1u) return s;
        s += 2u;
    }
}
DEVINL unsigned st_scatter_index(unsigned i, unsigned n, unsigned stride) { return stride == 1u ? i : (unsigned)(((unsigned long long)i * stride) % n); }
__global__ __launch_bounds__(64, 4) void mtr_k_dp2_quads(K2Args a, StagedArgs s)
{
    __shared__ unsigned long long s_cnt[CNT_N];
    const int lane = lane_id();
    if (lane < CNT_N) s_cnt[lane] = 0ull;
    if (st_staged_overflowed(a)) return;
    K2Ctx c;
    c.a = &a; c.wc = s_cnt;
    c.sc = a.scratch + (size_t)blockIdx.x * a.scratch_per_wave;
    c.y = k2_layout(a.Lmax, a.cells_cap);
    c.lds_keys = nullptr; c.seeds = nullptr; c.stage = nullptr; c.ties = nullptr; c.fresh = nullptr;
    st_dp2_waves_body(c, a, s);
    const unsigned nq = (unsigned)(uni(s.quad_cls[ST_QCLASSES]) >> 2);
    if (nq == 0u) { wc_flush(s_cnt, a.counters); return; }
    Wq wq; wq_init(wq, nq);
    const unsigned q_stride = s.pass_shuffle ? st_scatter_stride(nq) : 1u;
    for (;;) {
        const int wi = wq_next(ST_WQ(s, ST_Q_QUAD), nq, wq);
        if (wi < 0) break;
        const int slot0 = (int)st_scatter_index((unsigned)wi, nq, q_stride) << 2;
        DpQuad q; q.n = 0;
        int items[4], kk[4];
        int maxrows = 0;
#pragma unroll
        for (int g = 0; g < 4; g++) {
            const int di = uni(s.sorted[slot0 + g]);
            items[g] = di;
            const StDpItem *d = s.dp + (di >= 0 ? di : uni(s.sorted[slot0]));
            const int rd = uni(d->rd);
            q.pk[g] = a.b.packed + uni64(a.b.woff[rd]);
            q.wlim[g] = (long long)a.packed_words - uni64(a.b.woff[rd]);
            q.base[g] = uni(d->qs); q.rows[g] = di >= 0 ? uni(d->rows) : 0; q.U[g] = uni(d->U);
            q.unit[g] = s.arena + uni64(d->unit_off);
            kk[g] = uni(d->pad[0]);
            if (di >= 0) { q.n = g + 1; maxrows = q.rows[g] > maxrows ? q.rows[g] : maxrows; }
        }
        const int C = DPQ_COLS(q.U[0]);
        if (DPQ_BLOCK_BYTES(C, maxrows) > c.y.cells) {
            for (int g = 0; g < q.n; g++) {
                const StDpItem *d = s.dp + items[g];
                c.rd = uni(d->rd); c.L = uni(a.b.lens[c.rd]); c.pk = a.b.packed + uni64(a.b.woff[c.rd]);
                RR r; rr_clear(r); r.period = q.U[g]; r.kmer = kk[g];
                dp_two_params_unit(c, q.base[g], q.base[g] + q.rows[g] - 1, r, q.unit[g]);
                int *o = s.dp_res + (size_t)items[g] * 16;
                if (lane == 0) {
                    o[0] = r.rep_start; o[1] = r.rep_end; o[2] = r.repeat_len; o[3] = r.period; o[4] = r.copies; o[5] = r.mat; o[6] = r.mis;
                    o[7] = r.ins; o[8] = r.del; o[9] = r.kmer; o[10] = r.G; o[11] = r.MM; o[12] = r.D;
                }
                loop_join();
            }
            loop_join();
            continue;
        }
        switch (C) {
        case 1: st_quad_run<1>(c, a, s, items, q, kk, maxrows); break;
        case 2: st_quad_run<2>(c, a, s, items, q, kk, maxrows); break;
        case 3: st_quad_run<3>(c, a, s, items, q, kk, maxrows); break;
        case 4: st_quad_run<4>(c, a, s, items, q, kk, maxrows); break;
        case 5: st_quad_run<5>(c, a, s, items, q, kk, maxrows); break;
        case 6: st_quad_run<6>(c, a, s, items, q, kk, maxrows); break;
        case 7: st_quad_run<7>(c, a, s, items, q, kk, maxrows); break;
        default: st_quad_run<8>(c, a, s, items, q, kk, maxrows); break;
        }
        loop_join();
    }
    wc_flush(s_cnt, a.counters);
}

DEVINL void st_list_rev_block(const K2Args &a, const StagedArgs &s, long long base)
{
    const long long slot = st_reserve(s, ST_SL_RB, s.kc_cap, 1u);
    if (slot < 0) set_status(a.status, DEV_ERR_STAGED_OVERFLOW);
    else if (lane_id() == 0) s.rb_items[slot] = base;
}
__global__ __launch_bounds__(64, MTR_WAVES_PER_SIMD) void mtr_k_select(K2Args a, StagedArgs s)
{
    __shared__ __attribute__((aligned(16))) int s_arena[MTR_ARENA_INTS];
    __shared__ unsigned long long s_cnt[CNT_N];
    int *s_keys = s_arena, *s_seeds = s_arena + K2_TAB_CAP, *s_stage = s_seeds + MTRC_MAX_SEEDS + 4;
    const int lane = lane_id();
    if (lane < CNT_N) s_cnt[lane] = 0ull;
    if (st_staged_overflowed(a)) return;
    K2Ctx c;
    c.a = &a; c.wc = s_cnt;
    c.sc = a.scratch + (size_t)blockIdx.x * a.scratch_per_wave;
    c.y = k2_layout(a.Lmax, a.cells_cap);
    c.lds_keys = (lds_int *)s_keys; c.seeds = (lds_int *)s_seeds; c.stage = (lds_int *)s_stage;
    c.ties = (int *)(c.sc + c.y.ties); c.fresh = c.ties + MTRC_MAX_TIEBREAKS;
    const bool quads = s.quad_min > 0;
    WqS wq; (void)wqs_init(wq, s, ST_SL_KC, s.kc_cap);
    for (;;) {
        const long long wi = wqs_next(s, 5, s.kc_cap, wq);
        if (wi < 0) break;
        const long long base = uni64(s.kc_items[wi]);
        const StItemHdr *h = (const StItemHdr *)(s.arena + base);
        const StEnt *en = (const StEnt *)(h + 1);
        int hv = 0;
        if (lane < 12) hv = ((const int32_t *)h)[lane];
        const int n_slots = lane_val(hv, 0), min_k = lane_val(hv, 3), rd = lane_val(hv, 5), qs = lane_val(hv, 7), qe = lane_val(hv, 8), item = lane_val(hv, 10);
        const unsigned run_mask = (unsigned)lane_val(hv, 1), found_mask = (unsigned)lane_val(hv, 2);
        const int rows = qe - qs + 1, nk = n_slots >> 1, stride = lane_val(hv, 11);
        uint8_t *slot0 = s.arena + base + (long long)sizeof(StItemHdr) + (long long)sizeof(StEnt) * n_slots;
        int Ue = 0, ke = min_k, dpi = -1;
        if (lane < n_slots && lane < 64) { Ue = en[lane].period; ke = en[lane].k; dpi = en[lane].dpi; }
        const bool has = Ue > 0;
        const bool fnd = has && ((found_mask >> (ke - min_k)) & 1u);
        if (n_slots > 64 || (n_slots & 1) || __ballot(fnd && dpi < 0) != 0ull) {
            set_status(a.status, DEV_ERR_STAGED_OVERFLOW);
            loop_join();
            continue;
        }
        c.rd = rd;
        int r0 = -1, r1 = -1, r2 = -1, r3 = -1, r4 = -1, r5 = -1, r6 = -1, r7 = -1, r8 = -1, r9 = -1, r10 = -1, r11 = -1, r12 = -1;
        if (fnd) {
            const int4 *o = (const int4 *)(s.dp_res + (size_t)(dpi & ~ST_DPI_DUP) * 16);
            const int4 v0 = o[0], v1 = o[1], v2 = o[2]; const int v3 = ((const int *)o)[12];
            r0 = v0.x; r1 = v0.y; r2 = v0.z; r3 = v0.w; r4 = v1.x; r5 = v1.y; r6 = v1.z; r7 = v1.w; r8 = v2.x; r9 = v2.y; r10 = v2.z; r11 = v2.w; r12 = v3;
            if (r3 != -1) { r9 = ke; r3 = Ue; }
        }
        {
            const bool memo = has && (!fnd || (dpi & ST_DPI_DUP));
            const unsigned long long mm = __ballot(memo);
            if (mm != 0ull) { wc_add(c.wc, CNT_MEMO_HITS, __popcll(mm)); wc_add(c.wc, CNT_MEMO_CELLS, wave_sum_i64(memo ? 2ll * (long long)rows * (long long)Ue : 0ll)); }
        }
        const int ki = lane, k = min_k + ki;
        const int s0 = (2 * ki) & 63, s1 = (2 * ki + 1) & 63;
        const bool in_k = ki < nk;
        const bool has0 = __shfl((int)has, s0, 64) != 0 && in_k, has1 = __shfl((int)has, s1, 64) != 0 && in_k;
        int c0 = -1, c1 = -1, c2 = -1, c3 = -1, c4 = -1, c5 = -1, c6 = -1, c7 = -1, c8 = -1, c9 = -1, c10 = -1, c11 = -1, c12 = -1, k_slot = -1;
        float k_ratio = -1.0f;
#define ST_SEL_DIR(HAS, SRC, E)                                                                                                                        \
        {                                                                                                                                              \
            const int t0 = __shfl(r0, SRC, 64), t1 = __shfl(r1, SRC, 64), t2 = __shfl(r2, SRC, 64), t3 = __shfl(r3, SRC, 64), t4 = __shfl(r4, SRC, 64),     \
                      t5 = __shfl(r5, SRC, 64), t6 = __shfl(r6, SRC, 64), t7 = __shfl(r7, SRC, 64), t8 = __shfl(r8, SRC, 64), t9 = __shfl(r9, SRC, 64),     \
                      t10 = __shfl(r10, SRC, 64), t11 = __shfl(r11, SRC, 64), t12 = __shfl(r12, SRC, 64);                                                  \
            const float q = (float)t5 / (float)(t5 + t6 + t7 + t8);                                                                                        \
            if ((HAS) && k_ratio < q && a.min_match_ratio <= q && MTRC_MIN_NUM_FREQ_UNIT < t4 && MTRC_MIN_PERIOD <= t3 && t3 < MTRC_MAX_PERIOD) {          \
                k_ratio = q; k_slot = (E);                                                                                                                 \
                c0 = t0; c1 = t1; c2 = t2; c3 = t3; c4 = t4; c5 = t5; c6 = t6; c7 = t7; c8 = t8; c9 = t9; c10 = t10; c11 = t11; c12 = t12;                 \
            }                                                                                                                                              \
        }
        ST_SEL_DIR(has0, s0, 2 * ki)
        ST_SEL_DIR(has1, s1, 2 * ki + 1)
#undef ST_SEL_DIR
        const bool run = in_k && ((run_mask >> ki) & 1u);
        if (trace_on(c, 2))
            for (int q = 0; q < nk; q++) if ((run_mask >> q) & 1u)
                trace_ev(c, 2, qs, qe, min_k + q, (int)((found_mask >> q) & 1u), 0, lane_val(c3, q), lane_val(c0, q), lane_val(c1, q), lane_val(c2, q), lane_val(c4, q), lane_val(c5, q), lane_val(c6, q), lane_val(c7, q), lane_val(c8, q));
        bool rev = false;
        {
            bool clear = false;
            if (!in_k || !((found_mask >> ki) & 1u)) clear = true;
            else if ((long long)c3 * (long long)rows > mtr_dev_wrap_dp_size) clear = true;
            else if (c3 == 0) clear = true;
            else { const int coverage = c2 / c3; rev = run && 5 <= coverage && coverage <= 20 && 5 < c3; }
            if (clear) { c0 = c1 = c2 = c3 = c4 = c5 = c6 = c7 = c8 = c9 = c10 = c11 = c12 = -1; }
        }
        const unsigned long long revm = __ballot(rev);
        long long ro = -1;
        if (revm != 0ull) {
            const unsigned n_rev = (unsigned)__popcll(revm);
            const long long ro0 = st_reserve_bytes(s, (long long)n_rev * ST_REV_BYTES);
            long long ri = -1;
            if (quads) { const long long r0l = st_reserve(s, ST_SL_REV, s.rev_cap, n_rev); ri = r0l < 0 ? -1 : r0l + (long long)mbcnt(revm); }
            else {
                for (unsigned long long m = revm; m != 0ull; m &= m - 1ull) {
                    const int l = first_lane(m);
                    const int rcls = st_cost_class(lane_val(c1, l) - lane_val(c0, l) + 1);
                    unsigned got = 0; if (lane == 0) got = atomicAdd(s.n_rev + rcls * ST_CLS_STRIDE, 1u); got = (unsigned)uni((int)got);
                    if (lane == l) ri = got < (unsigned)s.rev_cap ? (long long)got : -1;
                    loop_join();
                }
            }
            const bool bad = rev && (ro0 < 0 || ri < 0 || (quads && ri >= (long long)s.dp_cap));
            if (__ballot(bad) != 0ull) set_status(a.status, DEV_ERR_STAGED_OVERFLOW);
            else if (rev) {
                ro = ro0 + (long long)mbcnt(revm) * ST_REV_BYTES;
                StRev *rv = (StRev *)(s.arena + ro);
                const int rcls = quads ? 0 : st_cost_class(c1 - c0 + 1);
                rv->block = base; rv->k = k; rv->slot = k_slot; rv->leader = -1; rv->ri = (int32_t)ri;
                rv->rr[0] = c0; rv->rr[1] = c1; rv->rr[2] = c2; rv->rr[3] = c3; rv->rr[4] = c4; rv->rr[5] = c5; rv->rr[6] = c6; rv->rr[7] = c7; rv->rr[8] = c8;
                rv->rr[9] = c9; rv->rr[10] = c10; rv->rr[11] = c11; rv->rr[12] = c12; rv->rr[13] = 0;
                s.rev_items[(size_t)rcls * (size_t)s.rev_cap + (size_t)ri] = ro;
                if (quads) s.dp_bin[ri] = -1;
            }
        }
        StK *kt = (StK *)(slot0 + (long long)n_slots * stride);
        if (in_k) {
            StK *x = kt + ki;
            if (!run) { x->state = 0; x->slot = -1; x->rev_off = -1; }
            else {
                x->state = (rev && ro >= 0) ? 2 : 1; x->slot = k_slot; x->rev_off = ro;
                x->rr[0] = c0; x->rr[1] = c1; x->rr[2] = c2; x->rr[3] = c3; x->rr[4] = c4; x->rr[5] = c5; x->rr[6] = c6; x->rr[7] = c7; x->rr[8] = c8;
                x->rr[9] = c9; x->rr[10] = c10; x->rr[11] = c11; x->rr[12] = c12; x->rr[13] = 0;
            }
        }
        if (__ballot(rev && ro >= 0) != 0ull) { wave_sync_mem(); st_list_rev_block(a, s, base); loop_join(); continue; }
        {
            RR best; rr_clear(best);
            float best_ratio = -1.0f;
            int best_e = -1;
            for (int q = 0; q < nk; q++) {
                if (!((run_mask >> q) & 1u)) continue;
                RR cur;
                cur.rep_start = lane_val(c0, q); cur.rep_end = lane_val(c1, q); cur.repeat_len = lane_val(c2, q); cur.period = lane_val(c3, q); cur.copies = lane_val(c4, q);
                cur.mat = lane_val(c5, q); cur.mis = lane_val(c6, q); cur.ins = lane_val(c7, q); cur.del = lane_val(c8, q); cur.kmer = lane_val(c9, q);
                cur.G = lane_val(c10, q); cur.MM = lane_val(c11, q); cur.D = lane_val(c12, q);
                if (k2_better(a, best_ratio, cur)) { best_ratio = rr_ratio(cur); best = cur; best_e = lane_val(k_slot, q); }
            }
            if (k2_qualifies(best) && best_e >= 0) {
                unsigned ci = 0;
                if (lane == 0) ci = atomicAdd(s.n_cand, 1u);
                ci = (unsigned)uni((int)ci);
                if (ci >= (unsigned)s.cand_cap) set_status(a.status, DEV_ERR_STAGED_OVERFLOW);
                else {
// ... 581 lines not shown
```

### mtr_amd/csrc/mtr_abi.hip

```cpp
#include <hip/hip_runtime.h>
#include <algorithm>
#include <atomic>
#include <chrono>
#include <cstdio>
#include <cstdlib>
#include <cstring>
#include <memory>
#include <numeric>
#include <string>
#include <vector>

#include <mutex>

#include "../../include/mtr_hip.h"
#include "../../include/mtr_hip_test.h"
#include "mtr_common.h"
#include "file_state.h"
#include "k1_ranges.hip.inc"
#include "k2_units.hip.inc"
#include "k3_staged.hip.inc"
#include "dp_test.hip.inc"
#include "pack.hip.inc"
#include "records.hip.inc"
#include "chain.hip.inc"
// ... 3852 lines not shown
        if (o + need > capacity) return -1;
        memcpy(out + o, r, MTR_WIRE_HEADER_BYTES);
        const int up = (p + 3) & ~3;
        memcpy(out + o + MTR_WIRE_HEADER_BYTES, r->unit, (size_t)p);
        memset(out + o + MTR_WIRE_HEADER_BYTES + p, 0, (size_t)(up - p));
        memcpy(out + o + MTR_WIRE_HEADER_BYTES + up, r->unit_score, (size_t)p * 4);
        o += need;
    }
    return o;
}

extern "C" mtr_status mtr_process_batch(mtr_ctx *ctx, const uint8_t *bases, const int64_t *offsets, const int32_t *lens,
                                        int32_t n_reads, mtr_record **out_records, int32_t **out_counts, int64_t *out_total)
{
    mtr_status s = mtr_upload_batch(ctx, bases, offsets, lens, n_reads); if (s != MTR_OK) return s;
    s = mtr_run_resident(ctx); if (s != MTR_OK) return s;
    return mtr_fetch_results(ctx, out_records, out_counts, out_total);
}

extern "C" void mtr_free_results(mtr_record *records, int32_t *counts) { free(records); free(counts); }

extern "C" mtr_status mtr_get_bases_after_read(const mtr_ctx *ctx, int32_t read_idx, uint8_t out[2])
{
    if (!ctx || !out || read_idx < 0 || read_idx >= ctx->n_reads || ctx->after.size() < (size_t)ctx->n_reads * 2) return MTR_ERR_BAD_ARG;
    out[0] = ctx->after[(size_t)read_idx * 2]; out[1] = ctx->after[(size_t)read_idx * 2 + 1];
    return MTR_OK;
}

extern "C" mtr_status mtr_get_kernel_times(const mtr_ctx *ctx, mtr_kernel_time *out, int32_t n)
{
    if (!ctx || !out) return MTR_ERR_BAD_ARG;
    for (int i = 0; i < n && i < MTR_N_KERNEL_TIMES; i++) out[i] = ctx->kt[i];
    return MTR_OK;
}

extern "C" mtr_status mtr_get_counters(const mtr_ctx *ctx, int64_t *out, int32_t n)
{
    if (!ctx || !out) return MTR_ERR_BAD_ARG;
    for (int i = 0; i < n && i < CNT_N; i++) out[i] = (int64_t)ctx->counters[i];
    return MTR_OK;
}

extern "C" mtr_status mtr_test_ranges(mtr_ctx *ctx, int32_t **out_counts, int32_t **out_start, int32_t **out_end,
                                      int32_t **out_w, uint64_t **out_di_bits, int64_t *out_total)
{
    if (!ctx || !out_counts || !out_start || !out_end || !out_w || !out_di_bits) return MTR_ERR_BAD_ARG;
    if (ctx->n_reads <= 0) { ctx->err = "no batch uploaded"; return MTR_ERR_BAD_ARG; }
    HIPCHK(hipSetDevice(ctx->device));
    read_switches(ctx->sw);
    HIPCHK(hipMemsetAsync(ctx->d_status, 0, 4, ctx->stream));
    HIPCHK(hipMemsetAsync(ctx->d_counters, 0, sizeof(unsigned long long) * CNT_N, ctx->stream));
    mtr_status s = launch_k1(ctx); if (s != MTR_OK) return s;
    HIPCHK(hipStreamSynchronize(ctx->stream));
    float ms = 0; HIPCHK(hipEventElapsedTime(&ms, ctx->ev[0], ctx->ev[1])); ctx->kt[0].ms = ms; ctx->kt[0].launches = 1;
    s = check_status(ctx); if (s != MTR_OK) return s;
    const int n = ctx->n_reads;
    std::vector<int32_t> cnt((size_t)n), st((size_t)ctx->total_rcap), en((size_t)ctx->total_rcap), ww((size_t)ctx->total_rcap);
    std::vector<uint64_t> di((size_t)ctx->total_rcap);
    HIPCHK(copy_sync(ctx, cnt.data(), ctx->d_rcount, (size_t)n * 4, hipMemcpyDeviceToHost));
    HIPCHK(copy_sync(ctx, st.data(), ctx->d_rstart, st.size() * 4, hipMemcpyDeviceToHost));
    HIPCHK(copy_sync(ctx, en.data(), ctx->d_rend, en.size() * 4, hipMemcpyDeviceToHost));
    HIPCHK(copy_sync(ctx, ww.data(), ctx->d_rw, ww.size() * 4, hipMemcpyDeviceToHost));
    HIPCHK(copy_sync(ctx, di.data(), ctx->d_rdi, di.size() * 8, hipMemcpyDeviceToHost));
    int64_t total = 0; for (int i = 0; i < n; i++) total += cnt[(size_t)i];
    const size_t m = (size_t)std::max<int64_t>(total, 1);
    HostArray<int32_t> oc = host_array<int32_t>((size_t)n), os = host_array<int32_t>(m), oe = host_array<int32_t>(m), ow = host_array<int32_t>(m);
    HostArray<uint64_t> od = host_array<uint64_t>(m);
    if (!oc || !os || !oe || !ow || !od) return MTR_ERR_OOM;
    int64_t p = 0;
    for (int i = 0; i < n; i++) {
        oc[i] = cnt[(size_t)i];
        for (int t = 0; t < cnt[(size_t)i]; t++, p++) {
            size_t q = (size_t)ctx->roff[(size_t)i] + (size_t)t;
            os[p] = st[q]; oe[p] = en[q]; ow[p] = ww[q]; od[p] = di[q];
        }
    }
    *out_counts = oc.release(); *out_start = os.release(); *out_end = oe.release(); *out_w = ow.release(); *out_di_bits = od.release(); if (out_total) *out_total = total;
    return MTR_OK;
}

extern "C" mtr_status mtr_test_file_tail(mtr_ctx *ctx, uint16_t **out_tail, int64_t **out_tail_off, uint8_t **out_after)
{
    if (!ctx || !out_tail || !out_tail_off || !out_after) return MTR_ERR_BAD_ARG;
    if (ctx->n_reads <= 0) { ctx->err = "no batch uploaded"; return MTR_ERR_BAD_ARG; }
    HIPCHK(hipSetDevice(ctx->device));
    const size_t n = (size_t)ctx->n_reads;
    const int64_t entries = ctx->file_order ? ctx->tail_entries : 0;
    HostArray<uint16_t> tl = host_array<uint16_t>((size_t)std::max<int64_t>(entries, 1));
    HostArray<int64_t> to = host_array<int64_t>(n + 1);
    HostArray<uint8_t> af = host_array<uint8_t>(n * 2);
    if (!tl || !to || !af) return MTR_ERR_OOM;
    tl[0] = 0; memset(to.get(), 0, (n + 1) * 8); memset(af.get(), 0, n * 2);
    if (ctx->file_order) {
        HIPCHK(copy_sync(ctx, to.get(), ctx->d_tail_off, (n + 1) * 8, hipMemcpyDeviceToHost));
        if (entries > 0) HIPCHK(copy_sync(ctx, tl.get(), ctx->d_tail, (size_t)entries * 2, hipMemcpyDeviceToHost));
        if (ctx->after.size() >= n * 2) memcpy(af.get(), ctx->after.data(), n * 2);
    }
    ctx->kt[0].ms = ctx->file_order ? ctx->fo_tail_ms : 0; ctx->kt[0].launches = ctx->file_order ? ctx->fo_tail_launches : 0;
    *out_tail = tl.release(); *out_tail_off = to.release(); *out_after = af.release();
    return MTR_OK;
}

extern "C" mtr_status mtr_test_wrap_dp(mtr_ctx *ctx, int32_t n_tasks, const int32_t *read_idx, const int32_t *query_start,
                                       const int32_t *query_end, const uint8_t *units, const int32_t *unit_off,
                                       const int32_t *gain, const int32_t *mismatch, const int32_t *indel, int32_t *out8)
{
    if (!ctx || n_tasks <= 0 || !read_idx || !query_start || !query_end || !units || !unit_off || !gain || !mismatch || !indel || !out8) return MTR_ERR_BAD_ARG;
    if (ctx->n_reads <= 0) { ctx->err = "no batch uploaded"; return MTR_ERR_BAD_ARG; }
    HIPCHK(hipSetDevice(ctx->device));
    read_switches(ctx->sw);
    size_t cells = 1;
    for (int t = 0; t < n_tasks; t++) {
        int rd = read_idx[t];
        int U = unit_off[t + 1] - unit_off[t];
        if (rd < 0 || rd >= ctx->n_reads || query_start[t] < 0 || query_end[t] < query_start[t] || query_end[t] >= ctx->lens[(size_t)rd] || U <= 0 || U >= MTRC_MAX_PERIOD) { ctx->err = "bad DP task " + std::to_string(t); return MTR_ERR_BAD_ARG; }
        cells = std::max(cells, (size_t)(query_end[t] - query_start[t] + 1) * (size_t)(U + 1));
    }
    size_t per_wave = mtrc_align(cells + 256, 256), total = 0;
    int waves = pick_waves(ctx, n_tasks, 8, per_wave, &total);
    DBG("test_wrap_dp: %d tasks, cells %zu, waves %d, scratch %zu", n_tasks, cells, waves, total);
    mtr_status s = ensure_scratch(ctx, total); if (s != MTR_OK) return s;
    const size_t nt = (size_t)n_tasks;
    HIPCHK(ctx->d_t_i32.ensure((nt * 7 + 1) * 4)); HIPCHK(ctx->d_t_units.ensure((size_t)unit_off[n_tasks] + 16)); HIPCHK(ctx->d_t_out.ensure(nt * 8 * 4));
    int32_t *d_i32 = ctx->d_t_i32; uint8_t *d_units = ctx->d_t_units; int32_t *d_out = ctx->d_t_out;
    int32_t *d_rd = d_i32, *d_qs = d_i32 + nt, *d_qe = d_i32 + 2 * nt, *d_g = d_i32 + 3 * nt, *d_m = d_i32 + 4 * nt, *d_d = d_i32 + 5 * nt, *d_uo = d_i32 + 6 * nt;
    HIPCHK(copy_sync(ctx, d_rd, read_idx, nt * 4, hipMemcpyHostToDevice)); HIPCHK(copy_sync(ctx, d_qs, query_start, nt * 4, hipMemcpyHostToDevice));
    HIPCHK(copy_sync(ctx, d_qe, query_end, nt * 4, hipMemcpyHostToDevice)); HIPCHK(copy_sync(ctx, d_g, gain, nt * 4, hipMemcpyHostToDevice));
    HIPCHK(copy_sync(ctx, d_m, mismatch, nt * 4, hipMemcpyHostToDevice)); HIPCHK(copy_sync(ctx, d_d, indel, nt * 4, hipMemcpyHostToDevice));
    HIPCHK(copy_sync(ctx, d_uo, unit_off, (nt + 1) * 4, hipMemcpyHostToDevice)); HIPCHK(copy_sync(ctx, d_units, units, (size_t)unit_off[n_tasks], hipMemcpyHostToDevice));
    DpTestArgs a{};
    a.b = view(ctx); a.n_tasks = n_tasks; a.read_idx = d_rd; a.qs = d_qs; a.qe = d_qe; a.units = d_units; a.unit_off = d_uo;
    a.gain = d_g; a.mism = d_m; a.indel = d_d; a.out8 = d_out; a.scratch = ctx->d_scratch; a.scratch_per_wave = per_wave; a.cells_cap = cells;
    a.status = ctx->d_status; a.work_counter = ctx->d_work; a.counters = ctx->d_counters; a.dp16_max_rows = ctx->sw.dp16_max_rows;
    HIPCHK(hipMemsetAsync(ctx->d_status, 0, 4, ctx->stream));
    HIPCHK(hipMemsetAsync(ctx->d_work, 0, sizeof(unsigned), ctx->stream));
    HIPCHK(hipMemsetAsync(ctx->d_counters, 0, sizeof(unsigned long long) * CNT_N, ctx->stream));
    HIPCHK(hipEventRecord(ctx->ev[2], ctx->stream));
    DBG("test_wrap_dp: launching");
    hipLaunchKernelGGL(mtr_k_dp_test, dim3((unsigned)waves), dim3(64), 0, ctx->stream, a);
    HIPCHK(hipGetLastError());
    HIPCHK(hipEventRecord(ctx->ev[3], ctx->stream));
    HIPCHK(hipStreamSynchronize(ctx->stream));
    DBG("test_wrap_dp: kernel done");
    float ms = 0; HIPCHK(hipEventElapsedTime(&ms, ctx->ev[2], ctx->ev[3])); ctx->kt[1].ms = ms; ctx->kt[1].launches = 1;
    HIPCHK(copy_sync(ctx, ctx->counters, ctx->d_counters, sizeof(unsigned long long) * CNT_N, hipMemcpyDeviceToHost));
    HIPCHK(copy_sync(ctx, out8, d_out, nt * 8 * 4, hipMemcpyDeviceToHost));
    return check_status(ctx);
}

extern "C" mtr_status mtr_test_wrap_dp_pass(mtr_ctx *ctx, int32_t pass, int32_t n_groups, const int32_t *group_off, const int32_t *read_idx,
                                            const int32_t *query_start, const int32_t *query_end, const uint8_t *units, const int32_t *unit_off,
                                            const int32_t *gain, const int32_t *mismatch, const int32_t *indel, int32_t *out16)
{
    if (!ctx || pass < MTR_TEST_PASS_WAVE2P || pass > MTR_TEST_PASS_OCT1P || n_groups <= 0 || !group_off || !read_idx || !query_start || !query_end || !units || !unit_off ||
        !gain || !mismatch || !indel || !out16) return MTR_ERR_BAD_ARG;
    if (ctx->n_reads <= 0) { ctx->err = "no batch uploaded"; return MTR_ERR_BAD_ARG; }
    if (group_off[0] != 0) { ctx->err = "group_off[0] is not 0"; return MTR_ERR_BAD_ARG; }
    HIPCHK(hipSetDevice(ctx->device));
    read_switches(ctx->sw);
    const long long lim16 = ctx->sw.dp16_max_rows;
    const bool one_param = pass == MTR_TEST_PASS_FOUR1P || pass == MTR_TEST_PASS_OCT1P;
    const int max_members = pass == MTR_TEST_PASS_WAVE2P ? 1 : pass == MTR_TEST_PASS_OCT1P ? RQ_SLOTS : 4;
    auto refuse = [&](int g, int t, const char *why) {
        ctx->err = "bad DP pass task " + std::to_string(t) + " (group " + std::to_string(g) + "): " + why; return MTR_ERR_BAD_ARG;
    };
    auto size_ok = [&](long long U, long long rows) { return (U + 1) * rows + U < ctx->wrap_dp_size; };
    size_t cells = 1;
    int quad_cols = 0;
    for (int g = 0; g < n_groups; g++) {
        const int t0 = group_off[g], n = group_off[g + 1] - t0;
        if (t0 < 0 || n < 1 || n > max_members) return refuse(g, t0, "empty group, or more members than the pass takes");
        long long maxrows = 0, maxU = 0, sumU = 0;
        for (int t = t0; t < t0 + n; t++) {
            const int rd = read_idx[t];
            const long long U = (long long)unit_off[t + 1] - unit_off[t];
            if (rd < 0 || rd >= ctx->n_reads || query_start[t] < 0 || query_end[t] < query_start[t] || query_end[t] >= ctx->lens[(size_t)rd]) return refuse(g, t, "window outside its read");
            if (U <= 0 || U >= MTRC_MAX_PERIOD) return refuse(g, t, "unit length");
            const long long rows = (long long)query_end[t] - query_start[t] + 1;
            if (!size_ok(U, rows)) return refuse(g, t, "beyond WrapDPsize");
            switch (pass) {
            case MTR_TEST_PASS_WAVE2P: break;
            case MTR_TEST_PASS_Q4:
                if (U > 16) return refuse(g, t, "unit above 16 bases");
                if (rows > DP2P_MAX_ROWS || rows > lim16 || !size_ok(16, rows)) return refuse(g, t, "rows beyond dp_batch_fits");
                if (rd != read_idx[t0] || query_start[t] != query_start[t0] || query_end[t] != query_end[t0]) return refuse(g, t, "the units of a Q4 group share read and window");
                break;
            case MTR_TEST_PASS_QUAD2P:
                if (U > ST_QUMAX) return refuse(g, t, "unit above ST_QUMAX");
                if (rows > DP2P_MAX_ROWS || rows > lim16 || !DPQ_FITS(rows, U, 1, 3)) return refuse(g, t, "rows beyond DPQ_FITS");
                if (quad_cols == 0) quad_cols = DPQ_COLS(U);
                if (DPQ_COLS(U) != quad_cols) return refuse(g, t, "the tasks of a QUAD2P call are of one DPQ_COLS class");
                break;
            default: {
                const int G = gain[t], MM = mismatch[t], D = indel[t];
                if (!((G == 1 && MM == 1 && D == 3) || (G == 1 && MM == 3 && D == 1) || (G == 5 && MM == 1 && D == 1))) return refuse(g, t, "not one of the three parameter sets");
                if (U > ST_QUMAX) return refuse(g, t, "unit above ST_QUMAX");
                if (rows > lim16 || !DPQ_FITS(rows, U, G, D)) return refuse(g, t, "rows beyond DPQ_FITS");
                break; }
            }
            maxrows = std::max(maxrows, rows); maxU = std::max(maxU, U); sumU += U;
        }
        size_t block;
        switch (pass) {
        case MTR_TEST_PASS_WAVE2P: block = 2 * (size_t)maxrows * (size_t)(maxU + 1) + 64; break;
        case MTR_TEST_PASS_Q4: block = (size_t)maxrows * (size_t)sumU; break;
        case MTR_TEST_PASS_QUAD2P: block = DPQ_BLOCK_BYTES(DPQ_COLS(maxU), maxrows); break;
        default: block = (RQ_SLOTS / 4) * DPQP_BLOCK_BYTES(DPQ_COLS(maxU), maxrows); break;
        }
        cells = std::max(cells, block);
    }
    const size_t per_wave = mtrc_align(cells + 256, 256);
    if (per_wave > scratch_cap(ctx)) { ctx->err = "bad DP pass task: a group's cell block of " + std::to_string(cells) + " bytes exceeds the scratch cap"; return MTR_ERR_BAD_ARG; }
    size_t total = 0;
    const int waves = pick_waves(ctx, n_groups, 8, per_wave, &total);
    mtr_status s = ensure_scratch(ctx, total); if (s != MTR_OK) return s;
    const size_t nt = (size_t)group_off[n_groups], ng = (size_t)n_groups;
    HIPCHK(ctx->d_t_i32.ensure((nt * 7 + 1 + ng + 1) * 4)); HIPCHK(ctx->d_t_units.ensure((size_t)unit_off[nt] + 16)); HIPCHK(ctx->d_t_out.ensure(nt * 16 * 4));
    int32_t *d_i32 = ctx->d_t_i32; uint8_t *d_units = ctx->d_t_units; int32_t *d_out = ctx->d_t_out;
    int32_t *d_rd = d_i32, *d_qs = d_i32 + nt, *d_qe = d_i32 + 2 * nt, *d_g = d_i32 + 3 * nt, *d_m = d_i32 + 4 * nt, *d_d = d_i32 + 5 * nt, *d_uo = d_i32 + 6 * nt, *d_go = d_i32 + 7 * nt + 1;
    HIPCHK(copy_sync(ctx, d_rd, read_idx, nt * 4, hipMemcpyHostToDevice)); HIPCHK(copy_sync(ctx, d_qs, query_start, nt * 4, hipMemcpyHostToDevice));
    HIPCHK(copy_sync(ctx, d_qe, query_end, nt * 4, hipMemcpyHostToDevice)); HIPCHK(copy_sync(ctx, d_g, gain, nt * 4, hipMemcpyHostToDevice));
    HIPCHK(copy_sync(ctx, d_m, mismatch, nt * 4, hipMemcpyHostToDevice)); HIPCHK(copy_sync(ctx, d_d, indel, nt * 4, hipMemcpyHostToDevice));
    HIPCHK(copy_sync(ctx, d_uo, unit_off, (nt + 1) * 4, hipMemcpyHostToDevice)); HIPCHK(copy_sync(ctx, d_units, units, (size_t)unit_off[nt], hipMemcpyHostToDevice));
    HIPCHK(copy_sync(ctx, d_go, group_off, (ng + 1) * 4, hipMemcpyHostToDevice));
    DpPassArgs a{};
    a.t.b = view(ctx); a.t.n_tasks = (int32_t)nt; a.t.read_idx = d_rd; a.t.qs = d_qs; a.t.qe = d_qe; a.t.units = d_units; a.t.unit_off = d_uo;
    a.t.gain = d_g; a.t.mism = d_m; a.t.indel = d_d; a.t.out8 = d_out; a.t.scratch = ctx->d_scratch; a.t.scratch_per_wave = per_wave; a.t.cells_cap = cells;
    a.t.status = ctx->d_status; a.t.work_counter = ctx->d_work; a.t.counters = ctx->d_counters; a.t.dp16_max_rows = ctx->sw.dp16_max_rows;
    a.pass = pass; a.n_groups = n_groups; a.group_off = d_go; a.packed_words = ctx->packed_words;
    HIPCHK(hipMemsetAsync(ctx->d_status, 0, 4, ctx->stream));
    HIPCHK(hipMemsetAsync(ctx->d_work, 0, sizeof(unsigned), ctx->stream));
    HIPCHK(hipMemsetAsync(ctx->d_counters, 0, sizeof(unsigned long long) * CNT_N, ctx->stream));
    HIPCHK(hipMemsetAsync(d_out, 0, nt * 16 * 4, ctx->stream));
    const dim3 grid((unsigned)waves), block(64);
    if (pass == MTR_TEST_PASS_WAVE2P || pass == MTR_TEST_PASS_Q4) hipLaunchKernelGGL(mtr_k_dp_test_waves, grid, block, 0, ctx->stream, a);
    else if (one_param) hipLaunchKernelGGL(mtr_k_dp_test_rev, grid, block, 0, ctx->stream, a);
    else {
        typedef void (*quad_kernel)(DpPassArgs);
        static const quad_kernel by_cols[8] = { mtr_k_dp_test_quads<1>, mtr_k_dp_test_quads<2>, mtr_k_dp_test_quads<3>, mtr_k_dp_test_quads<4>,
                                                mtr_k_dp_test_quads<5>, mtr_k_dp_test_quads<6>, mtr_k_dp_test_quads<7>, mtr_k_dp_test_quads<8> };
        hipLaunchKernelGGL(by_cols[quad_cols - 1], grid, block, 0, ctx->stream, a);
    }
    HIPCHK(hipGetLastError());
    HIPCHK(hipStreamSynchronize(ctx->stream));
    HIPCHK(copy_sync(ctx, ctx->counters, ctx->d_counters, sizeof(unsigned long long) * CNT_N, hipMemcpyDeviceToHost));
    HIPCHK(copy_sync(ctx, out16, d_out, nt * 16 * 4, hipMemcpyDeviceToHost));
    return check_status(ctx);
}

extern "C" mtr_status mtr_alignments(mtr_ctx *ctx, int32_t n, const int32_t *read_idx, const mtr_record *records,
                                     uint8_t **out_ops, int64_t **out_off, int32_t **out_end)
{
    if (!ctx || n < 0 || (n > 0 && (!read_idx || !records)) || !out_ops || !out_off || !out_end) return MTR_ERR_BAD_ARG;
    if (ctx->n_reads <= 0) { ctx->err = "no batch uploaded"; return MTR_ERR_BAD_ARG; }
    { mtr_status w = mtr_wait(ctx); if (w != MTR_OK && w != MTR_ERR_DP_TOO_LARGE) return w; }
    HIPCHK(hipSetDevice(ctx->device));
    read_switches(ctx->sw);
    HostArray<int64_t> off = host_array<int64_t>((size_t)n + 1);
    if (!off) return MTR_ERR_OOM;
    off[0] = 0;
    if (n == 0) { *out_ops = host_array<uint8_t>(1).release(); *out_off = off.release(); *out_end = host_array<int32_t>(2).release(); return MTR_OK; }
    const size_t nt = (size_t)n;
    std::vector<int32_t> h((nt * 6) + nt + 1);
    int32_t *h_rd = h.data(), *h_rs = h_rd + nt, *h_re = h_rs + nt, *h_g = h_re + nt, *h_m = h_g + nt, *h_d = h_m + nt, *h_uo = h_d + nt;
    std::vector<uint8_t> units; std::vector<int64_t> cap_off(nt + 1, 0);
    size_t cells = 1;
    for (int t = 0; t < n; t++) {
        const mtr_record &r = records[t];
        const int rd = read_idx[t], U = r.rep_period, rows = r.rep_end - r.rep_start + 1;
        if (rd < 0 || rd >= ctx->n_reads || U <= 0 || U >= MTRC_MAX_PERIOD || rows <= 0 || r.rep_start < 0 || r.rep_end > ctx->lens[(size_t)rd]) {
            ctx->err = "bad alignment task " + std::to_string(t); return MTR_ERR_BAD_ARG;
        }
        h_rd[t] = rd; h_rs[t] = r.rep_start; h_re[t] = r.rep_end; h_g[t] = r.match_gain; h_m[t] = r.mismatch_penalty; h_d[t] = r.indel_penalty;
        h_uo[t] = (int32_t)units.size();
        for (int j = 0; j < U; j++) { const char ch = r.unit[j]; units.push_back(ch == 'A' ? 0 : ch == 'C' ? 1 : ch == 'G' ? 2 : 3); }
        const size_t max_del = (size_t)std::max(r.match_gain, 1) * (size_t)rows / (size_t)std::max(r.indel_penalty, 1);
        cap_off[(size_t)t + 1] = cap_off[(size_t)t] + (int64_t)(((size_t)rows + max_del + (size_t)U + 64 + 3) & ~(size_t)3);
        cells = std::max(cells, (size_t)rows * (size_t)(U + 1));
    }
    h_uo[n] = (int32_t)units.size();
    const size_t per_wave = mtrc_align(cells + 256, 256);
    size_t total = 0;
    const int waves = pick_waves(ctx, n, 8, per_wave, &total);
    mtr_status s = ensure_scratch(ctx, total); if (s != MTR_OK) return s;
    const size_t ops_bytes = (size_t)cap_off[nt];
    HIPCHK(ctx->d_al_i32.ensure(h.size() * 4)); HIPCHK(ctx->d_al_len.ensure(nt * 4)); HIPCHK(ctx->d_al_units.ensure(units.size() + 16));
    HIPCHK(ctx->d_al_ops.ensure(ops_bytes + 16)); HIPCHK(ctx->d_al_off.ensure((nt + 1) * 8)); HIPCHK(ctx->d_al_ends.ensure(nt * 8));
    int32_t *d_i32 = ctx->d_al_i32;
    HIPCHK(hipMemcpyAsync(d_i32, h.data(), h.size() * 4, hipMemcpyHostToDevice, ctx->stream));
    HIPCHK(hipMemcpyAsync(ctx->d_al_units, units.data(), units.size(), hipMemcpyHostToDevice, ctx->stream));
    HIPCHK(hipMemcpyAsync(ctx->d_al_off, cap_off.data(), (nt + 1) * 8, hipMemcpyHostToDevice, ctx->stream));
    AlignArgs a{};
    a.b = view(ctx); a.n_tasks = n;
    a.read_idx = d_i32; a.rep_start = d_i32 + nt; a.rep_end = d_i32 + 2 * nt; a.gain = d_i32 + 3 * nt; a.mism = d_i32 + 4 * nt; a.indel = d_i32 + 5 * nt;
    a.unit_off = d_i32 + 6 * nt; a.units = ctx->d_al_units;
    a.ops = ctx->d_al_ops; a.ops_off = ctx->d_al_off; a.ops_len = ctx->d_al_len; a.ends = ctx->d_al_ends;
    a.scratch = ctx->d_scratch; a.scratch_per_wave = per_wave; a.cells_cap = cells;
    a.status = ctx->d_status; a.work_counter = ctx->d_work; a.counters = ctx->d_counters; a.dp16_max_rows = ctx->sw.dp16_max_rows;
    HIPCHK(hipMemsetAsync(ctx->d_status, 0, 4, ctx->stream));
    HIPCHK(hipMemsetAsync(ctx->d_work, 0, sizeof(unsigned), ctx->stream));
    hipLaunchKernelGGL(mtr_k_align, dim3((unsigned)waves), dim3(64), 0, ctx->stream, a);
    HIPCHK(hipGetLastError());
    std::vector<int32_t> len(nt);
    std::vector<uint8_t> raw(ops_bytes);
    HostArray<int32_t> ends = host_array<int32_t>(nt * 2);
    if (!ends) return MTR_ERR_OOM;
    HIPCHK(hipMemcpyAsync(ends.get(), ctx->d_al_ends, nt * 8, hipMemcpyDeviceToHost, ctx->stream));
    HIPCHK(hipMemcpyAsync(len.data(), ctx->d_al_len, nt * 4, hipMemcpyDeviceToHost, ctx->stream));
    HIPCHK(hipMemcpyAsync(raw.data(), ctx->d_al_ops, ops_bytes, hipMemcpyDeviceToHost, ctx->stream));
    HIPCHK(hipStreamSynchronize(ctx->stream));
    { mtr_status st = check_status(ctx); if (st != MTR_OK && !(st == MTR_ERR_DP_TOO_LARGE && ctx->run_status == MTR_ERR_DP_TOO_LARGE)) return st; }
    for (int t = 0; t < n; t++) off[(size_t)t + 1] = off[(size_t)t] + len[(size_t)t];
    HostArray<uint8_t> ops = host_array<uint8_t>((size_t)std::max<int64_t>(off[nt], 1));
    if (!ops) return MTR_ERR_OOM;
    for (int t = 0; t < n; t++) memcpy(ops.get() + off[(size_t)t], raw.data() + cap_off[(size_t)t], (size_t)len[(size_t)t]);
    for (int t = 0; t < n; t++) ends[2 * t] = records[t].rep_start - 1 + ends[2 * t];
    *out_ops = ops.release(); *out_off = off.release(); *out_end = ends.release();
    return MTR_OK;
}

extern "C" mtr_status mtr_set_trace(mtr_ctx *ctx, int32_t max_events)
{
    if (!ctx || max_events < 0) return MTR_ERR_BAD_ARG;
    HIPCHK(hipSetDevice(ctx->device));
    ctx->d_trace.release(); ctx->trace_cap = 0;
    if (max_events > 0) { HIPCHK(ctx->d_trace.alloc((size_t)max_events * 16 * 4)); ctx->trace_cap = max_events; }
    return MTR_OK;
}

extern "C" mtr_status mtr_get_trace(mtr_ctx *ctx, int32_t **out_events, int64_t *out_n)
{
    if (!ctx || !out_events || !out_n) return MTR_ERR_BAD_ARG;
    HIPCHK(hipSetDevice(ctx->device));
    unsigned n = 0;
    HIPCHK(copy_sync(ctx, &n, ctx->d_trace_n, 4, hipMemcpyDeviceToHost));
    if ((int64_t)n > ctx->trace_cap) n = (unsigned)ctx->trace_cap;
    HostArray<int32_t> ev = host_array<int32_t>((size_t)std::max(1u, n) * 16);
    if (!ev) return MTR_ERR_OOM;
    if (n > 0) HIPCHK(copy_sync(ctx, ev.get(), ctx->d_trace, (size_t)n * 16 * 4, hipMemcpyDeviceToHost));
    *out_events = ev.release(); *out_n = n;
    return MTR_OK;
}

#include "gather.hip.inc"
```

Before: 295,500.

## Pack eight small-unit DP tasks per wave with 8-lane segments

```diff
diff --git a/mtr_amd/__init__.py b/mtr_amd/__init__.py
--- a/mtr_amd/__init__.py
+++ b/mtr_amd/__init__.py
@@ -1523,7 +1523,7 @@
                                               g.ctypes.data, m.ctypes.data, d.ctypes.data, out.ctypes.data), "mtr_test_wrap_dp")
         return out
 
-    DP_PASSES = {"WAVE2P": 0, "Q4": 1, "QUAD2P": 2, "FOUR1P": 3, "OCT1P": 4}
+    DP_PASSES = {"WAVE2P": 0, "Q4": 1, "QUAD2P": 2, "FOUR1P": 3, "OCT1P": 4, "OCT2P": 5}
 
     def test_wrap_dp_pass(self, dp_pass: str, groups):
         tasks = [t for g in groups for t in g]
diff --git a/mtr_amd/csrc/device_util.hip.inc b/mtr_amd/csrc/device_util.hip.inc
--- a/mtr_amd/csrc/device_util.hip.inc
+++ b/mtr_amd/csrc/device_util.hip.inc
@@ -241,7 +241,7 @@
 DEVINL unsigned long long clk() { return 0ull; }
 DEVINL void wc_time(unsigned long long *, int, unsigned long long) {}
 #endif
-#ifdef MTR_PROFILE_WALK_FMT
+#if defined(MTR_PROFILE_WALK_FMT) || defined(MTR_PROFILE_DP2_CLASS)
 #define wc_time_aux(wc, which, t0) do { } while (0)
 #else
 #define wc_time_aux(wc, which, t0) wc_time(wc, which, t0)
diff --git a/mtr_amd/csrc/dp_quad.hip.inc b/mtr_amd/csrc/dp_quad.hip.inc
--- a/mtr_amd/csrc/dp_quad.hip.inc
+++ b/mtr_amd/csrc/dp_quad.hip.inc
@@ -23,23 +23,44 @@
 #define DPQP_DP_BYTES(C, maxrows) DPQP_DP_BYTES_G(16, C, maxrows)
 #define DPQP_BLOCK_BYTES(C, maxrows) (4 * DPQP_DP_BYTES(C, maxrows))
 
-template <int C, int GL = 16, int SC = DPQ_SCALE>
-DEVINL void dp_forward2p_g16(const DpQuad &q, int G0, int MM0, int D0, int G1, int MM1, int D1, uint8_t *cells, int maxrows, int (&best)[4][2][3])
+struct DpLanes {
+    const uint32_t *pk; long long wlim; int base, rows, U; const uint8_t *unit;
+};
+#define DPO_BLOCK_BYTES(C, maxrows) (8 * DPQ_DP_BYTES_G(8, C, maxrows))
+DEVINL void scan_max_u32_x2_row8(unsigned &a, unsigned &b)
 {
-    static_assert(C >= 1 && C <= 8 && (GL == 16 || GL == 64) && (SC == 1 || SC == 4), "columns per lane, lanes per DP, score scale");
+    unsigned s, t;
+#define MTR_SCAN_STEP(ctrl) \
+    s = (unsigned)__builtin_amdgcn_update_dpp(0, (int)a, ctrl, 0xf, 0xf, false); \
+    t = (unsigned)__builtin_amdgcn_update_dpp(0, (int)b, ctrl, 0xf, 0xf, false); \
+    a = s > a ? s : a; b = t > b ? t : b;
+    MTR_SCAN_STEP(0x111) MTR_SCAN_STEP(0x112) MTR_SCAN_STEP(0x114)
+#undef MTR_SCAN_STEP
+}
+template <int C, int GL = 16, int SC = DPQ_SCALE, class Q = DpQuad, class B = int[4][2][3]>
+DEVINL void dp_forward2p_g16(const Q &q, int G0, int MM0, int D0, int G1, int MM1, int D1, uint8_t *cells, int maxrows, B &best)
+{
+    static_assert(C >= 1 && C <= 8 && (GL == 16 || GL == 64 || (GL == 8 && C <= 4 && SC == 4)) && (SC == 1 || SC == 4), "columns per lane, lanes per DP, score scale");
     constexpr int NG = 64 / GL;
-    const int lane = lane_id();
+    int lane = lane_id();
+    if (GL == 8) asm volatile("" : "+v"(lane));
     const int g = lane / GL, l = lane % GL;
     unsigned Gpk = SC * ((unsigned)G0 | ((unsigned)G1 << 16)), MMpk = SC * ((unsigned)MM0 | ((unsigned)MM1 << 16)), Dpk = SC * ((unsigned)D0 | ((unsigned)D1 << 16));
     unsigned ONE = 0x00010001u, TWO = 0x00020002u, FOUR = 0x00040004u, SEL_HI = 0x07060100u, C8 = 0x00080008u;
     asm volatile("" : "+v"(ONE), "+v"(TWO), "+v"(FOUR), "+v"(SEL_HI), "+v"(C8));
     unsigned SEL_K0 = 0x0c040100u, SEL_K1 = 0x0c040302u, SEL_S = 0x05040100u, SEL_LO = 0x05040100u, SEL_P1 = 0x07060302u, K4N = ~0x00040004u;
     asm volatile("" : "+s"(MMpk), "+s"(Dpk), "+s"(SEL_K0), "+s"(SEL_K1), "+s"(SEL_S), "+s"(SEL_LO), "+s"(SEL_P1), "+s"(K4N));
-    int Ul = q.U[0], basel = q.base[0], rowsl = q.rows[0]; const uint8_t *up_ = q.unit[0]; const uint32_t *pkl = q.pk[0]; long long wl = q.wlim[0];
-    if (g == 1) { Ul = q.U[1]; basel = q.base[1]; rowsl = q.rows[1]; up_ = q.unit[1]; pkl = q.pk[1]; wl = q.wlim[1]; }
-    if (g == 2) { Ul = q.U[2]; basel = q.base[2]; rowsl = q.rows[2]; up_ = q.unit[2]; pkl = q.pk[2]; wl = q.wlim[2]; }
-    if (g == 3) { Ul = q.U[3]; basel = q.base[3]; rowsl = q.rows[3]; up_ = q.unit[3]; pkl = q.pk[3]; wl = q.wlim[3]; }
-    if (g >= q.n) { Ul = 0; rowsl = 0; }
+    int Ul, basel, rowsl; const uint8_t *up_; const uint32_t *pkl; long long wl;
+    if constexpr (GL == 8) {
+        Ul = q.U; basel = q.base; rowsl = q.rows; up_ = q.unit; pkl = q.pk; wl = q.wlim;
+        if (rowsl <= 0) { Ul = 0; rowsl = 0; }
+    } else {
+        Ul = q.U[0]; basel = q.base[0]; rowsl = q.rows[0]; up_ = q.unit[0]; pkl = q.pk[0]; wl = q.wlim[0];
+        if (g == 1) { Ul = q.U[1]; basel = q.base[1]; rowsl = q.rows[1]; up_ = q.unit[1]; pkl = q.pk[1]; wl = q.wlim[1]; }
+        if (g == 2) { Ul = q.U[2]; basel = q.base[2]; rowsl = q.rows[2]; up_ = q.unit[2]; pkl = q.pk[2]; wl = q.wlim[2]; }
+        if (g == 3) { Ul = q.U[3]; basel = q.base[3]; rowsl = q.rows[3]; up_ = q.unit[3]; pkl = q.pk[3]; wl = q.wlim[3]; }
+        if (g >= q.n) { Ul = 0; rowsl = 0; }
+    }
     unsigned ubw[2] = { 0x04040404u, 0x04040404u };
     unsigned Kc[C], KGc[C];
 #pragma unroll
@@ -72,8 +93,12 @@
     for (int c = 0; c < NBK; c++) { bk0[c] = 0u; bk1[c] = 0u; }
     unsigned wrapv = 0u;
     int next_done = maxrows + 1;
-#pragma unroll
-    for (int h = 0; h < NG; h++) { const int r = h < q.n ? q.rows[h] : 0; if (r < next_done) next_done = r; }
+    if constexpr (GL == 8) next_done = uni(-wave_max_i32(-rowsl));
+    else {
+#pragma unroll
+        for (int h = 0; h < NG; h++) { const int r = h < q.n ? q.rows[h] : 0; if (r < next_done) next_done = r; }
+    }
+    const unsigned long long seg_heads = GL == 8 ? 0x0101010101010101ull : 0ull;
     if (rowsl <= 0) { ubw[0] = 0x04040404u; ubw[1] = 0x04040404u; }
     uint8_t *crow = cells + (size_t)g * DPQ_DP_BYTES_G(GL, C, maxrows) + (size_t)l * C;
     int i = 1;
@@ -103,8 +128,11 @@
                 if (i > next_done) {
                     if (i > rowsl) { ubw[0] = 0x04040404u; ubw[1] = 0x04040404u; }
                     next_done = maxrows + 1;
-#pragma unroll
-                    for (int h = 0; h < NG; h++) { const int r = h < q.n ? q.rows[h] : 0; if (r >= i && r < next_done) next_done = r; }
+                    if constexpr (GL == 8) next_done = uni(-wave_max_i32(-(rowsl >= i ? rowsl : maxrows + 1)));
+                    else {
+#pragma unroll
+                        for (int h = 0; h < NG; h++) { const int r = h < q.n ? q.rows[h] : 0; if (r >= i && r < next_done) next_done = r; }
+                    }
                 }
                 const unsigned xi = __builtin_amdgcn_ubfe(wcur, (unsigned)bsh, 2u);
                 const unsigned inv_i = 0xFFFFu - (unsigned)i;
@@ -112,7 +140,8 @@
                 bool mt[C], nh[C];
                 unsigned sprev = 0u;
                 bool nhp = true;
-                const unsigned diag0 = GL == 16 ? (unsigned)row_shift_up1((int)P[C - 1], (int)wrapv) : (unsigned)shift_up1((int)P[C - 1], (int)wrapv);
+                unsigned diag0 = GL != 64 ? (unsigned)row_shift_up1((int)P[C - 1], (int)wrapv) : (unsigned)shift_up1((int)P[C - 1], (int)wrapv);
+                if (GL == 8) diag0 = lane0 ? wrapv : diag0;
 #pragma unroll
                 for (int c = 0; c < C; c++) {
                     const unsigned diag = c == 0 ? diag0 : P[c - 1];
@@ -127,14 +156,15 @@
                     nhp = nhp && !m; nh[c] = nhp;
                     sprev = sc;
                 }
-                const unsigned long long hm = __ballot(!nhp);
+                const unsigned long long hm = __ballot(!nhp) | seg_heads;
                 const unsigned seg = (unsigned)mbcnt(hm >> 1);
                 const unsigned sout = sprev + Dlane;
                 unsigned k0 = __builtin_amdgcn_perm(seg, sout, SEL_K0);
                 unsigned k1 = __builtin_amdgcn_perm(seg, sout, SEL_K1);
-                if (GL == 16) scan_max_u32_x2_row16(k0, k1); else scan_max_u32_x2(k0, k1);
+                if (GL == 8) scan_max_u32_x2_row8(k0, k1); else if (GL == 16) scan_max_u32_x2_row16(k0, k1); else scan_max_u32_x2(k0, k1);
                 const unsigned S = __builtin_amdgcn_perm(k1, k0, SEL_S);
-                const unsigned e = (GL == 16 ? (unsigned)row_shift_up1((int)S, 0) : (unsigned)shift_up1((int)S, 0)) - Dlane;
+                unsigned e = (GL != 64 ? (unsigned)row_shift_up1((int)S, 0) : (unsigned)shift_up1((int)S, 0)) - Dlane;
+                if (GL == 8) e = lane0 ? 0u : e;
                 unsigned f[8];
 #pragma unroll
                 for (int c = C; c < 8; c++) f[c] = 0u;
@@ -228,8 +258,11 @@
             const bool take = (ov > v) || (ov == v && ov > 0 && (oi < vi || (oi == vi && oj < vj)));
             if (take) { v = ov; vi = oi; vj = oj; }
         }
-#pragma unroll
-        for (int h = 0; h < NG; h++) { best[h][d][0] = lane_val(v, GL * h) / SC; best[h][d][1] = lane_val(vi, GL * h); best[h][d][2] = lane_val(vj, GL * h); }
+        if constexpr (GL == 8) { best[d][0] = v / SC; best[d][1] = vi; best[d][2] = vj; }
+        else {
+#pragma unroll
+            for (int h = 0; h < NG; h++) { best[h][d][0] = lane_val(v, GL * h) / SC; best[h][d][1] = lane_val(vi, GL * h); best[h][d][2] = lane_val(vj, GL * h); }
+        }
     }
 }
 
diff --git a/mtr_amd/csrc/dp_test.hip.inc b/mtr_amd/csrc/dp_test.hip.inc
--- a/mtr_amd/csrc/dp_test.hip.inc
+++ b/mtr_amd/csrc/dp_test.hip.inc
@@ -129,6 +129,51 @@
     wc_flush(s_cnt, a.t.counters);
 }
 
+__global__ __launch_bounds__(64, 4) void mtr_k_dp_test_octs(DpPassArgs a)
+{
+    __shared__ unsigned long long s_cnt[CNT_N];
+    const int lane = lane_id();
+    if (lane < CNT_N) s_cnt[lane] = 0ull;
+    uint8_t *cells = a.t.scratch + (size_t)blockIdx.x * a.t.scratch_per_wave;
+    for (;;) {
+        const int grp = next_work_item(a.t.work_counter);
+        if (grp >= a.n_groups) break;
+        const int t0 = uni(a.group_off[grp]), n = uni(a.group_off[grp + 1]) - t0;
+        DpLanes q;
+        {
+            const bool on = (lane >> 3) < n;
+            const int tg = t0 + (on ? (lane >> 3) : 0);
+            const int rd = a.t.read_idx[tg], uo = a.t.unit_off[tg];
+            const long long wo = a.t.b.woff[rd];
+            q.pk = a.t.b.packed + wo; q.wlim = a.packed_words - wo;
+            q.base = a.t.qs[tg]; q.rows = on ? a.t.qe[tg] - q.base + 1 : 0; q.U = on ? a.t.unit_off[tg + 1] - uo : 0;
+            q.unit = a.t.units + uo;
+        }
+        const int maxrows = uni(wave_max_i32(q.rows)), umax = uni(wave_max_i32(q.U));
+        const int C = (umax + 7) >> 3;
+        int best[2][3];
+        st_fwd2p_oct(C, q, cells, maxrows, best);
+        wave_sync_mem();
+        const int bestl = st_oct_best_lanes(best);
+#pragma unroll 1
+        for (int g = 0; g < n; g++) {
+            const int tg = t0 + g;
+            const int rd = uni(a.t.read_idx[tg]), qs = uni(a.t.qs[tg]), U = uni(a.t.unit_off[tg + 1]) - uni(a.t.unit_off[tg]);
+            for (int p = 0; p < 2; p++) {
+                const int bk[3] = { lane_val(bestl, 8 * g + 3 * p), lane_val(bestl, 8 * g + 3 * p + 1), lane_val(bestl, 8 * g + 3 * p + 2) };
+                DpRes o;
+                dpt_traceback<1>(a, a.t.b.packed + uni64(a.t.b.woff[rd]), qs, U, cells + (size_t)g * DPQ_DP_BYTES_G(8, C, maxrows), p, DPQ_ROW_BYTES_G(8, C), bk, o, s_cnt);
+                dpt_store(a, tg, p, qs, U, o);
+                loop_join();
+            }
+            loop_join();
+        }
+        wave_sync_mem();
+        loop_join();
+    }
+    wc_flush(s_cnt, a.t.counters);
+}
+
 __global__ __launch_bounds__(64, MTR_WAVES_PER_SIMD) void mtr_k_dp_test_rev(DpPassArgs a)
 {
     __shared__ unsigned long long s_cnt[CNT_N];
diff --git a/mtr_amd/csrc/k3_staged.hip.inc b/mtr_amd/csrc/k3_staged.hip.inc
--- a/mtr_amd/csrc/k3_staged.hip.inc
+++ b/mtr_amd/csrc/k3_staged.hip.inc
@@ -7,6 +7,8 @@
 #define ST_QSUB 8
 #define ST_NBINS (ST_QCLASSES * ST_QROWBINS * ST_QSUB)
 #define ST_QUMAX 128
+#define ST_OUMAX 32
+#define ST_OCLS0 (ST_QCLASSES - 2)
 
 struct StItemHdr {
     int32_t n_slots; uint32_t run_mask, found_mask; int32_t min_k, max_k;
@@ -585,6 +587,10 @@
             d->pad[0] = ke; d->pad[1] = cls;
             if (is_quad) {
                 int rb = ST_QROWBINS - 1 - (rows >> 3); if (rb < 0) rb = 0;
+                if (Ue <= ST_OUMAX) {
+                    int r8 = rows >> 3; if (r8 > ST_QROWBINS / 2 - 1) r8 = ST_QROWBINS / 2 - 1;
+                    rb = ((((Ue - 1) >> 3) & 1) ? 0 : ST_QROWBINS / 2) + ST_QROWBINS / 2 - 1 - r8;
+                }
                 const int bin = ((8 - DPQ_COLS(Ue)) * ST_QROWBINS + rb) * ST_QSUB + (int)(blockIdx.x & (ST_QSUB - 1));
                 s.dp_bin[di] = bin; s.dp_rank[di] = (int32_t)atomicAdd(s.bin_count + bin, 1u);
             } else {
@@ -628,9 +634,11 @@
         int off = 0;
         for (int c = 0; c < ST_QCLASSES; c++) {
             const int n = tot[(c + 1) * TPC - 1] - (c > 0 ? tot[c * TPC - 1] : 0);
+            if (!force && c == ST_OCLS0) off = (off + 7) & ~7;
             cls_start[c] = off; cls_n[c] = n;
             off += (n + 3) & ~3;
         }
+        if (!force) off = (off + 7) & ~7;
         cls_start[ST_QCLASSES] = off;
         const bool use = s.quad_min > 0 && (force || tot[1023] >= s.quad_min) && off <= s.sorted_cap;
         for (int c = 0; c <= ST_QCLASSES; c++) s.quad_cls[c] = use ? cls_start[c] : 0;
@@ -760,11 +768,22 @@
     dp_forward2p_g16<C>(q, 1, 1, 3, 1, 3, 1, cells, maxrows, best);
     wave_sync_mem();
     wc_time(c.wc, CYC_DP_FWD, t_f);
+#if defined(MTR_PROFILE) && defined(MTR_PROFILE_DP2_CLASS)
+    {
+        int umax = 0;
+        for (int g = 0; g < q.n; g++) umax = q.U[g] > umax ? q.U[g] : umax;
+        const int cls_ = C == 1 ? (umax <= 8 ? CNT_SPARE43 : CNT_SPARE44) : C == 2 ? CNT_SPARE45 : C <= 6 ? CNT_SPARE46 : CNT_SPARE47;
+        wc_add(c.wc, cls_, (long long)(clk() - t_f) + (1ll << 44));
+    }
+#endif
     if (lane == 0) {
         unsigned long long served = 0ull;
         for (int g = 0; g < q.n; g++) served += (unsigned long long)q.rows[g] * (unsigned long long)q.U[g];
         c.wc[CNT_QPASS_BYTES_DP2] += 4ull * (unsigned long long)maxrows * (unsigned long long)DPQ_ROW_BYTES(C);
         c.wc[CNT_QPASS_CELLS_DP2] += served;
+#ifndef MTR_PROFILE
+        c.wc[CNT_SPARE47] += 1ull;
+#endif
     }
     const unsigned long long t_b = clk();
 #pragma unroll
@@ -805,6 +824,102 @@
     wc_time(c.wc, CYC_DP_TB, t_b);
     wave_sync_mem();
 }
+DEVINL void st_fwd2p_oct(int C, const DpLanes &q, uint8_t *cells, int maxrows, int (&best)[2][3])
+{
+    switch (C) {
+    case 1: dp_forward2p_g16<1, 8>(q, 1, 1, 3, 1, 3, 1, cells, maxrows, best); break;
+    case 2: dp_forward2p_g16<2, 8>(q, 1, 1, 3, 1, 3, 1, cells, maxrows, best); break;
+    case 3: dp_forward2p_g16<3, 8>(q, 1, 1, 3, 1, 3, 1, cells, maxrows, best); break;
+    default: dp_forward2p_g16<4, 8>(q, 1, 1, 3, 1, 3, 1, cells, maxrows, best); break;
+    }
+}
+DEVINL int st_oct_best_lanes(const int (&best)[2][3])
+{
+    const int k = lane_id() & 7;
+    return k == 0 ? best[0][0] : k == 1 ? best[0][1] : k == 2 ? best[0][2] : k == 3 ? best[1][0] : k == 4 ? best[1][1] : best[1][2];
+}
+DEVINL bool st_oct_run(K2Ctx &c, const K2Args &a, const StagedArgs &s, int slot0)
+{
+    const int lane = lane_id();
+    const int di_l = s.sorted[slot0 + (lane >> 3)];
+    const unsigned long long present = __ballot(di_l >= 0);
+    if (present == 0ull) return true;
+    DpLanes q;
+    {
+        const StDpItem *d = s.dp + (di_l >= 0 ? di_l : lane_val(di_l, first_lane(present)));
+        const int rd = d->rd;
+        const long long wo = a.b.woff[rd];
+        q.pk = a.b.packed + wo; q.wlim = (long long)a.packed_words - wo;
+        q.base = d->qs; q.rows = di_l >= 0 ? d->rows : 0; q.U = di_l >= 0 ? d->U : 0;
+        q.unit = s.arena + d->unit_off;
+    }
+    const int maxrows = uni(wave_max_i32(q.rows)), umax = uni(wave_max_i32(q.U));
+    const int C = (umax + 7) >> 3;
+    if (DPO_BLOCK_BYTES(C, maxrows) > c.y.cells) return false;
+    uint8_t *cells = c.sc + c.y.codes;
+    int best[2][3];
+    const unsigned long long t_f = clk();
+    st_fwd2p_oct(C, q, cells, maxrows, best);
+    wave_sync_mem();
+    const int bestl = st_oct_best_lanes(best);
+    wc_time(c.wc, CYC_DP_FWD, t_f);
+#if defined(MTR_PROFILE) && defined(MTR_PROFILE_DP2_CLASS)
+    wc_add(c.wc, C == 1 ? CNT_SPARE43 : C == 2 ? CNT_SPARE44 : CNT_SPARE45, (long long)(clk() - t_f) + (1ll << 44));
+#endif
+    if (lane == 0) {
+        c.wc[CNT_QPASS_BYTES_DP2] += 8ull * (unsigned long long)maxrows * (unsigned long long)DPQ_ROW_BYTES_G(8, C);
+#ifndef MTR_PROFILE
+        c.wc[CNT_SPARE55] += 1ull;
+#endif
+    }
+    const unsigned long long t_b = clk();
+    const int rstride = DPQ_ROW_BYTES_G(8, C);
+    const size_t mbytes = DPQ_DP_BYTES_G(8, C, maxrows);
+#pragma unroll 1
+    for (int g = 0; g < 8; g++) {
+        const int di = uni(s.sorted[slot0 + g]);
+        if (di >= 0) {
+            const StDpItem *d = s.dp + di;
+            const int U = uni(d->U), qs = uni(d->qs), rows = uni(d->rows);
+            c.rd = uni(d->rd);
+            const uint32_t *pk = a.b.packed + uni64(a.b.woff[c.rd]);
+            const uint8_t *unit = s.arena + uni64(d->unit_off);
+            RR r; rr_clear(r); r.period = U; r.kmer = uni(d->pad[0]);
+            RR bestr; rr_clear(bestr);
+            float best_ratio = -1.0f;
+            long long tb = 0;
+            bool ok = true;
+            for (int p = 0; p < 2; p++) {
+                DpRes o; o.stop_i = 0; o.end_i = 0; o.mat = o.mis = o.ins = o.del = o.scanned = 0; o.end_j = 0;
+                const int bv = lane_val(bestl, 8 * g + 3 * p), bi = lane_val(bestl, 8 * g + 3 * p + 1), bj = lane_val(bestl, 8 * g + 3 * p + 2);
+                if (bv > 0) {
+                    dp_traceback<0, 1>(pk, qs, U, cells + (size_t)g * mbytes, p, rstride, bi, bj, nullptr, nullptr, nullptr, o, c.wc);
+                    if (o.stop_i < 0) { o.stop_i = 0; o.end_i = 0; o.mat = o.mis = o.ins = o.del = o.scanned = 0; ok = false; }
+                }
+                tb += (long long)(o.mat + o.mis + o.ins + o.del);
+                RR t = r;
+                apply_dp(t, qs, o, U, 1, p == 0 ? 1 : 3, p == 0 ? 3 : 1);
+                trace_ev(c, 3, qs, qs + rows - 1, U, trace_on(c, 3) ? unit_hash(unit, U) : 0, 1, p == 0 ? 1 : 3, p == 0 ? 3 : 1, t.rep_start, t.rep_end, t.repeat_len, t.copies, t.mat, t.mis, t.ins);
+                const float qq = rr_ratio(t);
+                if (best_ratio < qq) { bestr = t; best_ratio = qq; }
+                loop_join();
+            }
+            if (!ok) { dp_too_large(c); rr_clear(bestr); }
+            int *o = s.dp_res + (size_t)di * 16;
+            if (lane == 0) {
+                o[0] = bestr.rep_start; o[1] = bestr.rep_end; o[2] = bestr.repeat_len; o[3] = bestr.period; o[4] = bestr.copies; o[5] = bestr.mat; o[6] = bestr.mis;
+                o[7] = bestr.ins; o[8] = bestr.del; o[9] = bestr.kmer; o[10] = bestr.G; o[11] = bestr.MM; o[12] = bestr.D;
+                c.wc[CNT_DP_CALLS] += 2ull; c.wc[CNT_DP_CELLS] += 2ull * (unsigned long long)rows * (unsigned long long)U;
+                c.wc[CNT_DP_ROWS] += 2ull * (unsigned long long)rows; c.wc[CNT_TB_STEPS] += (unsigned long long)tb;
+                c.wc[CNT_QPASS_CELLS_DP2] += (unsigned long long)rows * (unsigned long long)U;
+            }
+        }
+        loop_join();
+    }
+    wc_time(c.wc, CYC_DP_TB, t_b);
+    wave_sync_mem();
+    return true;
+}
 DEVINL unsigned st_scatter_stride(unsigned n)
 {
     if (n < 4u) return 1u;
@@ -829,14 +944,20 @@
     c.y = k2_layout(a.Lmax, a.cells_cap);
     c.lds_keys = nullptr; c.seeds = nullptr; c.stage = nullptr; c.ties = nullptr; c.fresh = nullptr;
     st_dp2_waves_body(c, a, s);
-    const unsigned nq = (unsigned)(uni(s.quad_cls[ST_QCLASSES]) >> 2);
+    const int oct0 = uni(s.quad_cls[ST_OCLS0]);
+    const unsigned nq4 = (unsigned)(oct0 >> 2), nq = nq4 + (unsigned)((uni(s.quad_cls[ST_QCLASSES]) - oct0) >> 3);
     if (nq == 0u) { wc_flush(s_cnt, a.counters); return; }
     Wq wq; wq_init(wq, nq);
     const unsigned q_stride = s.pass_shuffle ? st_scatter_stride(nq) : 1u;
     for (;;) {
         const int wi = wq_next(ST_WQ(s, ST_Q_QUAD), nq, wq);
         if (wi < 0) break;
-        const int slot0 = (int)st_scatter_index((unsigned)wi, nq, q_stride) << 2;
+        const unsigned pi = st_scatter_index((unsigned)wi, nq, q_stride);
+        const bool oct = pi >= nq4;
+        const int slot0 = oct ? oct0 + (int)((pi - nq4) << 3) : (int)pi << 2;
+        bool fits = true;
+        if (oct) fits = st_oct_run(c, a, s, slot0);
+        else if (uni(s.sorted[slot0]) >= 0) {
         DpQuad q; q.n = 0;
         int items[4], kk[4];
         int maxrows = 0;
@@ -853,32 +974,35 @@
             kk[g] = uni(d->pad[0]);
             if (di >= 0) { q.n = g + 1; maxrows = q.rows[g] > maxrows ? q.rows[g] : maxrows; }
         }
-        const int C = DPQ_COLS(q.U[0]);
-        if (DPQ_BLOCK_BYTES(C, maxrows) > c.y.cells) {
-            for (int g = 0; g < q.n; g++) {
-                const StDpItem *d = s.dp + items[g];
-                c.rd = uni(d->rd); c.L = uni(a.b.lens[c.rd]); c.pk = a.b.packed + uni64(a.b.woff[c.rd]);
-                RR r; rr_clear(r); r.period = q.U[g]; r.kmer = kk[g];
-                dp_two_params_unit(c, q.base[g], q.base[g] + q.rows[g] - 1, r, q.unit[g]);
-                int *o = s.dp_res + (size_t)items[g] * 16;
-                if (lane == 0) {
-                    o[0] = r.rep_start; o[1] = r.rep_end; o[2] = r.repeat_len; o[3] = r.period; o[4] = r.copies; o[5] = r.mat; o[6] = r.mis;
-                    o[7] = r.ins; o[8] = r.del; o[9] = r.kmer; o[10] = r.G; o[11] = r.MM; o[12] = r.D;
-                }
-                loop_join();
-            }
-            loop_join();
-            continue;
-        }
-        switch (C) {
-        case 1: st_quad_run<1>(c, a, s, items, q, kk, maxrows); break;
-        case 2: st_quad_run<2>(c, a, s, items, q, kk, maxrows); break;
+        const int C = DPQ_COLS(q.U[0]) < 3 ? 3 : DPQ_COLS(q.U[0]);
+        fits = DPQ_BLOCK_BYTES(C, maxrows) <= c.y.cells;
+        if (fits) switch (C) {
         case 3: st_quad_run<3>(c, a, s, items, q, kk, maxrows); break;
         case 4: st_quad_run<4>(c, a, s, items, q, kk, maxrows); break;
         case 5: st_quad_run<5>(c, a, s, items, q, kk, maxrows); break;
         case 6: st_quad_run<6>(c, a, s, items, q, kk, maxrows); break;
         case 7: st_quad_run<7>(c, a, s, items, q, kk, maxrows); break;
         default: st_quad_run<8>(c, a, s, items, q, kk, maxrows); break;
+        }
+        }
+        if (!fits) {
+#pragma unroll 1
+            for (int g = 0; g < (oct ? 8 : 4); g++) {
+                const int di = uni(s.sorted[slot0 + g]);
+                if (di >= 0) {
+                    const StDpItem *d = s.dp + di;
+                    c.rd = uni(d->rd); c.L = uni(a.b.lens[c.rd]); c.pk = a.b.packed + uni64(a.b.woff[c.rd]);
+                    const int qs = uni(d->qs), rows = uni(d->rows);
+                    RR r; rr_clear(r); r.period = uni(d->U); r.kmer = uni(d->pad[0]);
+                    dp_two_params_unit(c, qs, qs + rows - 1, r, s.arena + uni64(d->unit_off));
+                    int *o = s.dp_res + (size_t)di * 16;
+                    if (lane == 0) {
+                        o[0] = r.rep_start; o[1] = r.rep_end; o[2] = r.repeat_len; o[3] = r.period; o[4] = r.copies; o[5] = r.mat; o[6] = r.mis;
+                        o[7] = r.ins; o[8] = r.del; o[9] = r.kmer; o[10] = r.G; o[11] = r.MM; o[12] = r.D;
+                    }
+                }
+                loop_join();
+            }
         }
         loop_join();
     }
diff --git a/mtr_amd/csrc/mtr_abi.hip b/mtr_amd/csrc/mtr_abi.hip
--- a/mtr_amd/csrc/mtr_abi.hip
+++ b/mtr_amd/csrc/mtr_abi.hip
@@ -4028,7 +4028,7 @@
                                             const int32_t *query_start, const int32_t *query_end, const uint8_t *units, const int32_t *unit_off,
                                             const int32_t *gain, const int32_t *mismatch, const int32_t *indel, int32_t *out16)
 {
-    if (!ctx || pass < MTR_TEST_PASS_WAVE2P || pass > MTR_TEST_PASS_OCT1P || n_groups <= 0 || !group_off || !read_idx || !query_start || !query_end || !units || !unit_off ||
+    if (!ctx || pass < MTR_TEST_PASS_WAVE2P || pass > MTR_TEST_PASS_OCT2P || n_groups <= 0 || !group_off || !read_idx || !query_start || !query_end || !units || !unit_off ||
         !gain || !mismatch || !indel || !out16) return MTR_ERR_BAD_ARG;
     if (ctx->n_reads <= 0) { ctx->err = "no batch uploaded"; return MTR_ERR_BAD_ARG; }
     if (group_off[0] != 0) { ctx->err = "group_off[0] is not 0"; return MTR_ERR_BAD_ARG; }
@@ -4036,7 +4036,7 @@
     read_switches(ctx->sw);
     const long long lim16 = ctx->sw.dp16_max_rows;
     const bool one_param = pass == MTR_TEST_PASS_FOUR1P || pass == MTR_TEST_PASS_OCT1P;
-    const int max_members = pass == MTR_TEST_PASS_WAVE2P ? 1 : pass == MTR_TEST_PASS_OCT1P ? RQ_SLOTS : 4;
+    const int max_members = pass == MTR_TEST_PASS_WAVE2P ? 1 : pass == MTR_TEST_PASS_OCT1P ? RQ_SLOTS : pass == MTR_TEST_PASS_OCT2P ? 8 : 4;
     auto refuse = [&](int g, int t, const char *why) {
         ctx->err = "bad DP pass task " + std::to_string(t) + " (group " + std::to_string(g) + "): " + why; return MTR_ERR_BAD_ARG;
     };
@@ -4067,6 +4067,10 @@
                 if (quad_cols == 0) quad_cols = DPQ_COLS(U);
                 if (DPQ_COLS(U) != quad_cols) return refuse(g, t, "the tasks of a QUAD2P call are of one DPQ_COLS class");
                 break;
+            case MTR_TEST_PASS_OCT2P:
+                if (U > ST_OUMAX) return refuse(g, t, "unit above ST_OUMAX");
+                if (rows > DP2P_MAX_ROWS || rows > lim16 || !DPQ_FITS(rows, U, 1, 3)) return refuse(g, t, "rows beyond DPQ_FITS");
+                break;
             default: {
                 const int G = gain[t], MM = mismatch[t], D = indel[t];
                 if (!((G == 1 && MM == 1 && D == 3) || (G == 1 && MM == 3 && D == 1) || (G == 5 && MM == 1 && D == 1))) return refuse(g, t, "not one of the three parameter sets");
@@ -4081,6 +4085,7 @@
         case MTR_TEST_PASS_WAVE2P: block = 2 * (size_t)maxrows * (size_t)(maxU + 1) + 64; break;
         case MTR_TEST_PASS_Q4: block = (size_t)maxrows * (size_t)sumU; break;
         case MTR_TEST_PASS_QUAD2P: block = DPQ_BLOCK_BYTES(DPQ_COLS(maxU), maxrows); break;
+        case MTR_TEST_PASS_OCT2P: block = DPO_BLOCK_BYTES((maxU + 7) / 8, maxrows); break;
         default: block = (RQ_SLOTS / 4) * DPQP_BLOCK_BYTES(DPQ_COLS(maxU), maxrows); break;
         }
         cells = std::max(cells, block);
@@ -4111,6 +4116,7 @@
     const dim3 grid((unsigned)waves), block(64);
     if (pass == MTR_TEST_PASS_WAVE2P || pass == MTR_TEST_PASS_Q4) hipLaunchKernelGGL(mtr_k_dp_test_waves, grid, block, 0, ctx->stream, a);
     else if (one_param) hipLaunchKernelGGL(mtr_k_dp_test_rev, grid, block, 0, ctx->stream, a);
+    else if (pass == MTR_TEST_PASS_OCT2P) hipLaunchKernelGGL(mtr_k_dp_test_octs, grid, block, 0, ctx->stream, a);
     else {
         typedef void (*quad_kernel)(DpPassArgs);
         static const quad_kernel by_cols[8] = { mtr_k_dp_test_quads<1>, mtr_k_dp_test_quads<2>, mtr_k_dp_test_quads<3>, mtr_k_dp_test_quads<4>,
```

New measurement: 303,900, median of 6. 1.03x the previous value.
